# liortalker/MindTheEdge

Measured on AMD Instinct MI355X. Metric: training images/sec, PackNet-SAN+edge-loss 384x1280 bf16, higher is better.
Workload: dtype bf16; 1 GPU; T8: PackNet-SAN + silog + 4-scale depth-edge loss training step, 384x1280, 8 frames/GPU, dropout 0.5, flip 0.5; global_batch=8, height=384, width=1280, parallelism=single GPU

## Files before the change

include/mte_kernels.h:

```cpp
#ifndef MTE_KERNELS_H
#define MTE_KERNELS_H

#ifdef __cplusplus
extern "C" {
#endif

typedef struct ihipStream_t* mte_stream_t;

#define MTE_OK 0
#define MTE_ERR_ARG (-1)
#define MTE_ERR_LAUNCH (-2)
#define MTE_ERR_UNSUPPORTED (-3)
#define MTE_DT_BF16 0
#define MTE_DT_F32 1

#define MTE_CONV_ACCUMULATE 1
#define MTE_CONV_SOLO 2
int mte_conv2d_igemm(const void* x, long ldx, const void* wpack, const float* bias, void* y, long ldy, int out_f32,
                     int B, int H, int W, int Cin_p, int N, int KH, int KW, int dtype,
                     float* workspace, long workspace_elems, int accumulate, mte_stream_t stream);
int mte_conv2d_igemm_unshuffle(const void* x, long ldx, const void* wpack, void* y, long ldy,
                               int B, int H, int W, int Cin_p, int N, int KH, int KW, int dtype, int accumulate, mte_stream_t stream);
#define MTE_OPT_GN_PREZEROED 0
#define MTE_OPT_LOSS_PREZEROED 1
#define MTE_OPT_HANDOFF_FENCES 2
#define MTE_OPT_WGRAD_SHARES_CHIP 3
int mte_set_option(int option, int value);
#define MTE_DEVERR_GN_CLUSTER_FWD 1
#define MTE_DEVERR_GN_CLUSTER_BWD 2
#define MTE_DEVERR_IMAGE_RESAMPLE 4
int mte_device_error_init(void);
int mte_device_error_poll(void);
int mte_conv2d_wgrad(const void* x, long ldx, const void* dy, long ldy, float* dw_stage, int stage_parts, int* parts_out,
                     int B, int H, int W, int Cin_p, int N, int KH, int KW, int dtype, mte_stream_t stream);
int mte_conv2d_wgrad_nine_tap(int H, int W, int Cin_p, int N, int KH, int KW, int dtype);
int mte_pack_conv_weights(const float* w_oihw, void* wfwd, void* wbwd, int Cout, int Cin, int KH, int KW,
                          int Cin_p, int Cout_p, int dtype, mte_stream_t stream);
typedef struct { const float* w; void* wf; void* wb; void* pf; void* pb; int Cout, Cin, taps, Cin_p; int end_f, end_b, end_pf, end_pb; } mte_pack_job;
int mte_pack_conv_weights_multi(const void* jobs, int njobs, int dtype, mte_stream_t stream);
int mte_pack_conv_weights_bwd(const void* wfwd, void* wbwd, int Cout, int KH, int KW, int Cin_p, int dtype, mte_stream_t stream);
int mte_unpack_conv_wgrad(float* dw_stage, int parts, float* dw_oihw, int Cout, int Cin, int KH, int KW, int Cin_p, mte_stream_t stream);
int mte_colsum(const void* y, long ld, long M, int N, float* out, int dtype, mte_stream_t stream);

int mte_conv2d_patch_supported(int W, int Cin_p, int N, int KH, int KW, int dtype);
int mte_conv2d_patch_wgrad_supported(int W, int Cin_p, int N, int KH, int KW, int dtype);
long mte_conv2d_patch_pack_elems(int Cin_p, int N, int KH, int KW);
int mte_conv2d_patch_repack(const void* wgeneric, void* wpatch, int Cin_p, int N, int KH, int KW, mte_stream_t stream);
int mte_conv2d_patch_fwd(const void* x, long ldx, const void* wpatch, const float* bias, void* y, long ldy,
                         int B, int H, int W, int Cin_p, int N, int KH, int KW, int accumulate, mte_stream_t stream);
int mte_conv2d_patch_wgrad(const void* x, long ldx, const void* dy, long lddy, float* dw_stage, int stage_parts, int* parts_out,
                           int B, int H, int W, int Cin_p, int N, int KH, int KW, mte_stream_t stream);
long mte_conv2d_patch_fwd_gn_elems(int B, int H, int W);
int mte_conv2d_patch_fwd_gn(const void* x, long ldx, const void* wpatch, const float* bias, void* y, long ldy, int B, int H, int W, int Cin_p, int N, int KH, int KW,
                            int accumulate, float* rec, long rec_elems, int* tiles_per_sample_out, mte_stream_t stream);

int mte_conv2d_stem_supported(int W, int Cin_p, int N, int KH, int KW, int dtype);
int mte_conv2d_stem_fwd(const void* x, long ldx, const void* wf, const float* bias, void* y, long ldy,
                        int B, int H, int W, int N, int KH, int KW, mte_stream_t stream);
int mte_conv2d_stem_wgrad(const void* x, long ldx, const void* dy, long lddy, float* dw_stage, int stage_parts, int* parts_out,
                          int B, int H, int W, int N, int KH, int KW, mte_stream_t stream);

long mte_gn_stats_elems(int B);
int mte_gn_stats(const void* y1, long ld1, const void* y2, long ld2, const float* scale2, double* stats,
                 int B, int HW, int C, int dtype, mte_stream_t stream);
int mte_gn_stats_from_records(const float* rec, int tiles_per_sample, double* stats, int B, mte_stream_t stream);
int mte_gn_fwd_is_single_pass(int HW, int C, int has_y2, int dtype);
int mte_gn_fwd_is_single_pass_b(int B, int HW, int C, int has_y2, int dtype);
int mte_gn_elu_fwd(const void* y1, long ld1, const void* y2, long ld2, const float* scale2, double* stats, int stats_ready,
                   const float* gamma, const float* beta, void* z, long ldz,
                   int B, int HW, int C, float eps, int dtype, mte_stream_t stream);
int mte_gn_elu_bwd(const void* dz, long lddz, const void* y1, long ld1, const void* y2, long ld2, const float* scale2,
                   const double* stats, const float* gamma, const float* beta, float* red,
                   void* d1, long ldd1, void* d2, long ldd2, float* dgamma, float* dbeta, float* dbias,
                   int B, int HW, int C, float eps, int dtype, mte_stream_t stream);
int mte_gn_tail_fwd(const void* y1, long ld1, const double* stats1, const float* gamma1, const float* beta1,
                    const void* y2, long ld2, const float* scale2, void* t, long ldt, double* stats_t,
                    const float* gamma_t, const float* beta_t, void* z, long ldz,
                    int B, int HW, int C, float eps, int dtype, mte_stream_t stream);

int mte_pack3d_fwd(const void* x, long ldx, const float* w3, const float* b3, void* out, long ldo,
                   int B, int H, int W, int C, int dtype, mte_stream_t stream);
int mte_pack3d_bwd_data(const void* dout, long ldo, const float* w3, void* dx, long lddx,
                        int B, int H, int W, int C, int dtype, mte_stream_t stream);
int mte_pack3d_bwd_weight(const void* x, long ldx, const void* dout, long ldo, float* dwb,
                          int B, int H, int W, int C, int dtype, mte_stream_t stream);
int mte_unpack3d_fwd(const void* x, long ldx, const float* w3, const float* b3, void* out, long ldo,
                     int B, int H, int W, int C, int dtype, mte_stream_t stream);
int mte_unpack3d_bwd_data(const void* dout, long ldo, const float* w3, void* dx, long lddx,
                          int B, int H, int W, int C, int dtype, mte_stream_t stream);
int mte_unpack3d_bwd_weight(const void* x, long ldx, const void* dout, long ldo, float* dwb,
                            int B, int H, int W, int C, int dtype, mte_stream_t stream);

int mte_fold_pack_weights(const float* W, const float* K3, const float* b, const float* b3, float* Wf, float* bf,
                          int Co, int D, int k, mte_stream_t stream);
int mte_unfold_pack_wgrad(const float* dWf, const float* dbf, const float* W, const float* K3, const float* b3,
                          float* dW, float* dk3b, int Co, int D, int k, int accumulate, mte_stream_t stream);
int mte_pixel_shuffle(const void* src, long lds_, void* dst, long ldd, int B, int H, int W, int C, int dir, int dtype, mte_stream_t stream);
int mte_copy_rect(const void* src, long lds_, int Hs, int Ws, int sy, int sx, void* dst, long ldd, int Hd, int Wd, int dy, int dx,
                  int B, int h, int w, int C, int mode, int dtype, mte_stream_t stream);
typedef struct { const void* src; long lds_; int Hs, Ws, sy, sx; void* dst; long ldd; int Hd, Wd, dy, dx, h, w, mode; } mte_rect_op;
int mte_copy_rects(const void* ops, int n, int B, int C, int dtype, mte_stream_t stream);

int mte_invdepth_fwd(const void* x, long ldx, const float* w, const float* bias, float* out,
                     int B, int H, int W, int C, float min_depth, int dtype, mte_stream_t stream);
int mte_invdepth_bwd_data(const float* w, const float* inv_out, const float* dout, float* dlogit,
                          void* dx, long lddx, int B, int H, int W, int C, float min_depth, int dtype, mte_stream_t stream);
long mte_invdepth_bwd_weight_workspace_elems(int C);
int mte_invdepth_bwd_weight(const void* x, long ldx, const float* dlogit, float* dwb, float* records,
                            int B, int H, int W, int C, int dtype, mte_stream_t stream);

int mte_rank1_conv_fwd(const float* inv, const float* w, long w_stride, void* y, long ldy, int B, int h, int wl, int N, int dtype, mte_stream_t stream);
int mte_rank1_conv_bwd_data(const void* dy, long lddy, const float* w, long w_stride, float* dinv, int B, int h, int wl, int N, int accumulate, int dtype,
                            mte_stream_t stream);
int mte_upsample2_f32(const float* inv, float* out, int B, int h, int wl, mte_stream_t stream);
int mte_conv2d_patch_fwd_rank1_ok(const float* bias, long ldx, int B, int H, int W, int Cin_p, int N);
int mte_conv2d_patch_fwd_rank1(const void* x, long ldx, const void* wpatch, const float* bias, void* y, long ldy, int B, int H, int W, int Cin_p, int N,
                               const float* inv, const float* w1, long w1_stride, mte_stream_t stream);
int mte_conv2d_patch_fwd_plus1x1(const void* x, long ldx, const void* wpatch, const float* bias, void* y, long ldy, int B, int H, int W, int Cin_p, int N,
                                 const void* x2, long ldx2, const void* wpatch2, int C2, mte_stream_t stream);
long mte_rank1_conv_bwd_records_elems(int N);
int mte_rank1_conv_bwd_weight(const void* dy, long lddy, const float* inv, float* dw, long dw_stride, float* records,
                              int B, int h, int wl, int N, int dtype, mte_stream_t stream);
int mte_nchw_to_nhwc(const float* src, void* dst, long ldd, int B, int C, int H, int W, int Cp, int flip_w, int dtype, mte_stream_t stream);
int mte_upsample_inv_fwd(const float* inv, void* dst, long ldd, int B, int h, int w, int dtype, mte_stream_t stream);
int mte_upsample_inv_bwd(const void* dsrc, long lds_, float* dinv, int B, int h, int w, int accumulate, int dtype, mte_stream_t stream);
int mte_copy_channels(const void* src, long lds_, void* dst, long ldd, long npix, int C, int dtype, mte_stream_t stream);
int mte_split_record(const float* src, float* dst0, int n0, float* dst1, int n1, mte_stream_t stream);
int mte_add_channels(const void* a, long lda, const void* b, long ldb, void* out, long ldo, long npix, int C, int dtype, mte_stream_t stream);

typedef struct { const float* pred; const float* edge; const float* normal; const float* mask; float* gmap; float* dpred; int H; int W; } mte_edge_scale;
long mte_edge_loss_work_elems(const void* scales, int nscales, int B);
int mte_edge_loss_multi_fwd(const void* scales, int nscales, int B, int from_inv, int is_grad, int is_sigmoid, float thresh,
                            float weight, float pos_to_neg, const float* gt_depth, double* work, float* losses, float* coef,
                            float* silog_loss, float* silog_aux, mte_stream_t stream);
int mte_edge_loss_multi_bwd(const void* scales, int nscales, int B, int from_inv, int is_grad, int is_sigmoid, float thresh,
                            const float* coef, const float* gout, const float* gt_depth, const float* silog_aux, const float* silog_gout,
                            mte_stream_t stream);
typedef struct { const float* pred[2]; float* dpred[2]; const float* edge; const float* normal; int H; int W; } mte_edge_pair_scale;
long mte_edge_loss_pair_work_elems(const void* scales, int nscales, int B);
int mte_edge_loss_pair_fwd(const void* scales, int nscales, int B, float thresh, float weight, float pos_to_neg,
                           const float* gt_depth, double* work, float* losses, float* coef,
                           float* silog_loss, float* silog_aux, mte_stream_t stream);
int mte_edge_loss_pair_bwd(const void* scales, int nscales, int B, float thresh, const float* coef, const float* gout,
                           const float* gt_depth, const float* silog_aux, const float* silog_gout, mte_stream_t stream);
long mte_edge_loss_sums_elems(int B, int H, int W);
int mte_edge_loss_fwd(const float* pred, const float* edge, const float* normal, const float* mask, double* sums, float* gmap,
                      int B, int H, int W, int from_inv, int is_grad, int is_sigmoid, float thresh, mte_stream_t stream);
int mte_edge_loss_finalize(const double* sums, int B, long numel, float weight, float pos_to_neg, int has_mask,
                           float out_scale, float* loss_acc, float* loss_this, float* coef, mte_stream_t stream);
int mte_edge_loss_bwd(const float* pred, const float* edge, const float* normal, const float* mask, const float* coef, const float* gout,
                      float* dpred, int B, int H, int W, int from_inv, int is_grad, int is_sigmoid, float thresh, mte_stream_t stream);

long mte_edge_loss_kind_work_elems(int B, int H, int W);
int mte_edge_loss_kind_fwd(const float* pred, const float* edge, const float* normal, const float* mask, float* gmap, int B, int H, int W,
                           int kind, int dice, int from_inv, int is_grad, int is_sigmoid, float thresh, float weight, float pos_to_neg,
                           double* work, float* loss, float* coef, mte_stream_t stream);
int mte_edge_loss_kind_bwd(const float* pred, const float* edge, const float* normal, const float* mask, const float* coef, const float* gout,
                           float* dpred, int B, int H, int W, int kind, int dice, int from_inv, int is_grad, int is_sigmoid, float thresh,
                           mte_stream_t stream);

typedef struct { const float* pred; float* dpred; int H; int W; } mte_sup_scale;
long mte_supervised_loss_work_elems(const void* scales, int nscales, int B);
int mte_supervised_loss_fwd(const void* scales, int nscales, int B, const float* depth, int Hd, int Wd, int method, int sparse,
                            double* work, float* loss, float* scale_loss, float* coef, mte_stream_t stream);
int mte_supervised_loss_bwd(const void* scales, int nscales, int B, const float* depth, int Hd, int Wd, int method, int sparse,
                            const float* coef, const float* gout, mte_stream_t stream);
typedef struct { const float* src; float* dst; int h; int w; } mte_upsample_map;
int mte_upsample_nearest_fwd(const void* maps, int nmaps, int B, int H, int W, mte_stream_t stream);
int mte_upsample_nearest_bwd(const void* maps, int nmaps, int B, int H, int W, mte_stream_t stream);

int mte_resize_bilinear_fwd(const float* x, float* y, int B, int h, int w, int H, int W, mte_stream_t stream);
int mte_resize_bilinear_bwd(const float* dy, float* dx, int B, int h, int w, int H, int W, mte_stream_t stream);

int mte_silog_fwd(const float* inv, const float* depth, long n, double* sums, float out_scale, float* loss_acc, float* loss_this, float* aux, mte_stream_t stream);
int mte_silog_bwd(const float* inv, const float* depth, const float* aux, const float* gout, float* dinv, long n, int accumulate, mte_stream_t stream);

int mte_adam_step(float* p, const float* g, float* m, float* v, long n, float lr, float beta1, float beta2, float eps,
                  int step, float gscale, mte_stream_t stream);
int mte_adam_step_dev(float* p, const float* g, float* m, float* v, long n, const float* hyper, float beta1, float beta2, float eps,
                      float gscale, mte_stream_t stream);
int mte_adamw_step(float* p, const float* g, float* m, float* v, long n, float lr, float beta1, float beta2, float eps, float weight_decay,
                   int decoupled, int step, float gscale, mte_stream_t stream);
int mte_adamw_step_dev(float* p, const float* g, float* m, float* v, long n, const float* hyper, float beta1, float beta2, float eps,
                       float weight_decay, int decoupled, float gscale, mte_stream_t stream);
int mte_sgd_step(float* p, const float* g, float* buf, long n, float lr, float momentum, float dampening, float weight_decay, int nesterov,
                 int step, float gscale, mte_stream_t stream);
int mte_sgd_step_dev(float* p, const float* g, float* buf, long n, const float* hyper, float momentum, float weight_decay, int nesterov,
                     float gscale, mte_stream_t stream);

long mte_depth_metrics_workspace_bytes(int B);
int mte_depth_metrics(const float* gt, const float* pred, int B, int H, int W, int h, int w, int scale_mode, int garg_crop,
                      float min_depth, float max_depth, int use_gt_scale, void* workspace, long workspace_bytes,
                      float* out7, mte_stream_t stream);
int mte_post_process_inv_depth(const float* inv_depth, const float* inv_depth_flipped, float* out, int B, int H, int W,
                               int method, mte_stream_t stream);

int mte_dee_sobel_nms(const float* pred, float scale, unsigned char* normals_u8, float* nms, int B, int H, int W, mte_stream_t stream);
int mte_hysteresis_begin(const float* img, unsigned char* state, int* info, int B, int H, int W, double t_low, double t_high,
                         mte_stream_t stream);
int mte_hysteresis_propagate(unsigned char* state, int* flags, int sweeps, int B, int H, int W, mte_stream_t stream);
int mte_hysteresis_finish(const float* img, const unsigned char* state, const int* info, float* out, int B, int H, int W,
                          mte_stream_t stream);

long mte_chamfer_workspace_bytes(int B, int H, int W);
int mte_chamfer_distance(const float* im_pred, const float* im_gt, int B, int H, int W, double edge_to_edge_thresh,
                         void* workspace, long workspace_bytes, double* out, float* dist_map, float* cond_map, mte_stream_t stream);

int mte_canny_begin(const float* depth, int B, int H, int W, int n_pairs, const int* thresholds, unsigned* max_ws,
                    unsigned char* vis_u8, unsigned char* state, mte_stream_t stream);
int mte_resize_linear(const float* src, int B, int h, int w, float* dst, int H, int W, mte_stream_t stream);
int mte_canny_propagate(unsigned char* state, int* flags, int sweeps, int maps, int H, int W, mte_stream_t stream);
int mte_canny_finish(const unsigned char* state, float* edges, int maps, int H, int W, mte_stream_t stream);
int mte_canny_begin_fixed(const float* depth, int B, int H, int W, float min_depth, float max_depth, float factor, int n_pairs,
                          const int* thresholds, unsigned char* vis_u8, unsigned char* state, mte_stream_t stream);

long mte_edge_match_workspace_bytes(int B, int H, int W, int r2);
int mte_edge_match(const float* pred, const float* gt, const int* gt_of, int B, int Bg, int H, int W, int r2, const int* init_mate,
                   void* workspace, long workspace_bytes, int* result, int* mate_pred, mte_stream_t stream);

int mte_frame_depth_metrics(const double* gt, const float* pred, const unsigned char* mask_u8, int B, int H, int W,
                            double min_depth, double max_depth, int x0, int x1, int y0, int y1, double* out, long* counts, mte_stream_t stream);

int mte_sparsify_depth(const float* depth, void* feat, long ldf, unsigned char* mask, int B, int H, int W, int dtype, mte_stream_t stream);
long mte_sparse_site_list_workspace_elems(long npix);
int mte_sparse_site_list(const unsigned char* mask, long npix, int* sites, int* count, int* ws, mte_stream_t stream);
int mte_conv2d_igemm_sparse(const void* x, long ldx, const void* wpack, const float* bias, void* y, long ldy,
                            int B, int H, int W, int Cin_p, int N, int KH, int KW, int dtype,
                            const int* sites, const int* count, int accumulate, mte_stream_t stream);
int mte_sparse_maxpool3s2(const void* in, long ldi, const unsigned char* mask_in, void* out, long ldo, unsigned char* mask_out,
                          int B, int H, int W, int C, int dtype, mte_stream_t stream);
int mte_sparse_bn_relu(const void* a, long lda, const void* b, long ldb, const void* c, long ldc, const unsigned char* mask,
                       const float* gamma, const float* beta, const float* mean, const float* var, float eps,
                       void* out, long ldo, long npix, int C, int dtype, mte_stream_t stream);
int mte_san_fuse(const void* skip, long ld_skip, const void* sparse, long ld_sparse, const float* w, const float* bias,
                 void* out, long ldo, long npix, int C, int dtype, mte_stream_t stream);
int mte_sparse_bn_stats(const void* a, long lda, const void* b, long ldb, const void* c, long ldc, const unsigned char* mask,
                        double* sums, long npix, int C, int dtype, mte_stream_t stream);
int mte_sparse_bn_relu_bwd(const void* a, long lda, const void* b, long ldb, const void* c, long ldc, const void* out, long ldo,
                           const void* dout, long ldd, const unsigned char* mask, const float* gamma, const float* mean, const float* invstd,
                           const double* n_active, double* sums, void* dx, long ldx, long npix, int C, int dtype, mte_stream_t stream);
int mte_sparse_maxpool3s2_bwd(const void* in, long ldi, const unsigned char* mask_in, const void* dout, long ldd, void* din, long ldn,
                              int B, int H, int W, int C, int dtype, mte_stream_t stream);
int mte_san_fuse_bwd(const void* skip, long ld_skip, const void* dout, long ldd, const float* w, void* dskip, long ldk, double* sums,
                     long npix, int C, int dtype, mte_stream_t stream);
int mte_feat_l2(const void* a, long lda, const void* b, long ldb, double* sum, void* db, long ldg, const float* gscale, float inv_n,
                long npix, int C, int dtype, mte_stream_t stream);

int mte_edge_target_from_u8(const unsigned char* src, float* dst, long n, mte_stream_t stream);
int mte_normal_target_from_u8(const unsigned char* src, float* dst, long n, mte_stream_t stream);
int mte_resize_depth_preserve(const float* src, int B, int h, int w, float* dst, int H, int W, int* winner_ws, mte_stream_t stream);

int mte_resize_linear_u8(const unsigned char* src, int B, int h, int w, unsigned char* dst, int H, int W, mte_stream_t stream);
int mte_resize_nearest_f32(const float* src, int B, int h, int w, float* dst, int H, int W, mte_stream_t stream);

long mte_image_resample_work_bytes(int in_h, int in_w, int out_h, int out_w, int two_pass);
int mte_image_resample_u8(const unsigned char* src, long src_stride, int crop_x, int crop_y, int in_h, int in_w, unsigned char* dst,
                          int out_h, int out_w, const int* kk_h, const int* bounds_h, int ksize_h, const int* kk_v, const int* bounds_v,
                          int ksize_v, unsigned char* workspace, int two_pass, mte_stream_t stream);
int mte_color_jitter_u8_to_f32(const unsigned char* in, int B, int H, int W, const float* factors, const int* order, int any_contrast,
                               unsigned long long* luma_sums, float* out, float* out_original, mte_stream_t stream);

#define MTE_PREP_EDGE_U8 0
#define MTE_PREP_SPARSE_U16 1
#define MTE_PREP_SPARSE_F32 2
#define MTE_PREP_NORMAL_U8 3
#define MTE_BATCH_PREP_ROW_WORDS 12
int mte_batch_prep(const unsigned char* arena, long arena_bytes, const long* table_host, const long* table_dev, int n_maps, float* out,
                   long out_elems, int* work, long winner_elems, mte_stream_t stream);

long mte_lidar_perturb_work_bytes(int H, int W);
int mte_lidar_index(const float* depth, int H, int W, void* work, mte_stream_t stream);
int mte_lidar_perturb(const float* depth, int H, int W, int n, double scale_d0, const double* add_i, const double* add_j, const double* add_d,
                      void* work, mte_stream_t stream);
int mte_lidar_scatter(int H, int W, int n, const unsigned char* keep, int n_keep, float* out, const void* work, mte_stream_t stream);
int mte_lidar_project(const double* points, int N, const double* K, const float* depth_map, float* out, int H, int W, int* winner_ws,
                      mte_stream_t stream);

long mte_order_stats_work_bytes(int B);
int mte_order_stats_f32(const float* x, long stride, int B, long n, const int* k, int positive_only, float* out, int* count_out, void* work,
                        mte_stream_t stream);
int mte_colormap_u8(const float* x, int B, int H, int W, const float* divisor, const float* lo_hi, const unsigned char* table, unsigned char* out,
                    mte_stream_t stream);
int mte_d3r_count(const float* gt, const float* pred, int H, int W, const void* index_work, int n, const int* pairs, int P, int* count,
                  mte_stream_t stream);

#ifdef MTE_DEV
int mte_debug_set(int key, int value);
#endif

#ifdef __cplusplus
}
#endif
#endif
```

mindtheedge_amd/_build.py:

```python
import hashlib
import os
import subprocess
import sys
from concurrent.futures import ThreadPoolExecutor

CSRC = os.path.join(os.path.dirname(os.path.abspath(__file__)), "csrc")
LIB = os.path.join(CSRC, "libmte_hip.so")
SOURCES = ["conv_igemm.hip", "conv_igemm8.hip", "conv_wgrad9.hip", "tap_wgrad.hip", "conv_patch.hip", "conv_stem.hip", "norm_act.hip", "pack3d.hip", "pack_fold.hip", "heads_misc.hip", "optim.hip", "edge_loss.hip", "edge_loss_kinds.hip", "supervised_loss.hip", "eval_metrics.hip", "dee_post.hip", "chamfer.hip", "canny.hip", "edge_match.hip", "san.hip", "data_prep.hip", "batch_prep.hip", "eval_prep.hip", "image_prep.hip", "lidar_prep.hip", "depth_viz.hip"]
FLAGS = ["--offload-arch=gfx950", "-O3", "-fPIC", "-std=c++17", "-Wno-unused-value", "-ffp-contract=off"]


def _hipcc():
    for c in (os.environ.get("HIPCC"), "/opt/rocm/bin/hipcc", "hipcc"):
        if c and (os.path.isabs(c) and os.path.exists(c) or not os.path.isabs(c)):
            return c
    raise RuntimeError("hipcc not found")


def _digest(paths, extra=""):
    h = hashlib.sha256(extra.encode())
    for p in paths:
        with open(p, "rb") as f:
            h.update(f.read())
    return h.hexdigest()


def _stale(target, digest):
    stamp = target + ".sha256"
    if not (os.path.exists(target) and os.path.exists(stamp)):
        return True
    with open(stamp) as f:
        return f.read().strip() != digest


def _stamp(target, digest):
    with open(target + ".sha256", "w") as f:
        f.write(digest + "\n")


DEV_LIB = os.path.join(CSRC, "libmte_hip_dev.so")


def headers(csrc=CSRC):
    return sorted(os.path.join(csrc, f) for f in os.listdir(csrc) if f.endswith(".hpp"))


def build(force=False, verbose=False, dev=True):
    hipcc = _hipcc()
    hdrs = headers()
    os.makedirs(os.path.join(CSRC, "dev"), exist_ok=True)
    variants = [("", [], LIB)] + ([("dev", ["-DMTE_DEV"], DEV_LIB)] if dev else [])
    jobs = []
    for sub, extra, _ in variants:
        for s in SOURCES:
            src, obj = os.path.join(CSRC, s), os.path.join(CSRC, sub, s.replace(".hip", ".o"))
            dig = _digest([src] + hdrs, " ".join(FLAGS + extra))
            if force or _stale(obj, dig):
                jobs.append(([hipcc] + FLAGS + extra + ["-c", src, "-o", obj], obj, dig))

    def run(cmd):
        if verbose:
            print(" ".join(cmd), file=sys.stderr)
        r = subprocess.run(cmd, capture_output=True, text=True)
        if r.returncode != 0:
            raise RuntimeError("hipcc failed:\n%s\n%s" % (" ".join(cmd), r.stderr[-4000:]))

    def compile_one(job):
        cmd, obj, dig = job
        run(cmd)
        _stamp(obj, dig)

    if jobs:
        with ThreadPoolExecutor(max_workers=min(int(os.environ.get("MTE_BUILD_JOBS", "6")), len(jobs))) as ex:
            list(ex.map(compile_one, jobs))
    for sub, _, target in variants:
        objs = [os.path.join(CSRC, sub, s.replace(".hip", ".o")) for s in SOURCES]
        lib_dig = _digest(objs, "link")
        if force or _stale(target, lib_dig):
            run([hipcc, "--offload-arch=gfx950", "-shared", "-fPIC", "-o", target] + objs)
            _stamp(target, lib_dig)
    return LIB


if __name__ == "__main__":
    print(build(force="--force" in sys.argv, verbose=True))
```

mindtheedge_amd/_lib.py:

```python
import ctypes
import os
import re

_HERE = os.path.dirname(os.path.abspath(__file__))
HEADER = os.path.join(os.path.dirname(_HERE), "include", "mte_kernels.h")
DEV_LIB_PATH = os.path.join(_HERE, "csrc", "libmte_hip_dev.so")
_USE_DEV = bool(os.environ.get("MTE_USE_DEV_LIB"))
LIB_PATH = os.environ.get("MTE_LIB_PATH") or (DEV_LIB_PATH if _USE_DEV else os.path.join(_HERE, "csrc", "libmte_hip.so"))

_CTYPES = {"int": ctypes.c_int, "long": ctypes.c_long, "float": ctypes.c_float, "double": ctypes.c_double, "mte_stream_t": ctypes.c_void_p}
_ERRORS = {-1: "MTE_ERR_ARG (bad argument / unsupported shape)", -2: "MTE_ERR_LAUNCH (HIP launch failed)",
           -3: "MTE_ERR_UNSUPPORTED"}


class MteError(RuntimeError):
    pass


RETURNS = {}
QUERIES = ("mte_conv2d_patch_supported", "mte_conv2d_stem_supported", "mte_conv2d_patch_wgrad_supported", "mte_conv2d_wgrad_nine_tap", "mte_conv2d_patch_fwd_gn_elems", "mte_conv2d_patch_pack_elems", "mte_depth_metrics_workspace_bytes",
           "mte_chamfer_workspace_bytes", "mte_edge_match_workspace_bytes", "mte_edge_loss_sums_elems", "mte_gn_fwd_is_single_pass", "mte_gn_fwd_is_single_pass_b",
           "mte_edge_loss_work_elems", "mte_edge_loss_pair_work_elems", "mte_edge_loss_kind_work_elems", "mte_supervised_loss_work_elems", "mte_rank1_conv_bwd_records_elems", "mte_conv2d_patch_fwd_rank1_ok", "mte_gn_stats_elems", "mte_device_error_poll", "mte_invdepth_bwd_weight_workspace_elems", "mte_sparse_site_list_workspace_elems", "mte_image_resample_work_bytes", "mte_lidar_perturb_work_bytes", "mte_order_stats_work_bytes")


def parse_header(path=HEADER, dev=False):
    text = open(path).read()
    text = re.sub(r"/\*.*?\*/", "", text, flags=re.S)
    if not dev:
        text = re.sub(r"#ifdef MTE_DEV.*?#endif", "", text, flags=re.S)
    protos = {}
    for m in re.finditer(r"\b(int|long)\s+(mte_\w+)\s*\(([^)]*)\)\s*;", text):
        RETURNS[m.group(2)] = ctypes.c_long if m.group(1) == "long" else ctypes.c_int
        args = []
        for a in ([] if m.group(3).strip() in ("", "void") else m.group(3).split(",")):
            a = " ".join(a.split())
            if "*" in a:
                args.append((ctypes.c_void_p, a.split("*")[-1].strip()))
            else:
                ty, name = a.rsplit(" ", 1)
                args.append((_CTYPES[ty.replace("const ", "").strip()], name))
        protos[m.group(2)] = args
    return protos


class _Lib:
    def __init__(self, path=None, dev=None):
        self._dll = None
        self._path = path or LIB_PATH
        self._dev = (self._path == DEV_LIB_PATH) if dev is None else bool(dev)
        self._protos = parse_header(dev=self._dev)
        self._options = {}
        self._loaded = {}

    def load(self):
        if self._dll is None:
            if not os.path.exists(self._path):
                raise MteError("%s is not built (%s). Run `python -c 'import __graft_entry__ as g; g.build()'` "
                               "or `python mindtheedge_amd/_build.py`; there is no CPU/eager fallback." % (os.path.basename(self._path), self._path))
            import torch
            dll = self._loaded.get(self._path)
            if dll is None:
                dll = self._loaded[self._path] = ctypes.CDLL(self._path)
            for name, args in self._protos.items():
                fn = getattr(dll, name)
                fn.argtypes = [t for t, _ in args]
                fn.restype = RETURNS.get(name, ctypes.c_int)
            self._dll = dll
            for opt, val in self._options.items():
                dll.mte_set_option(opt, val)
        return self._dll

    def switch(self, path, dev):
        for k in [k for k in self.__dict__ if k.startswith("mte_")]:
            del self.__dict__[k]
        self._dll, self._path, self._dev = None, path, bool(dev)
        self._protos = parse_header(dev=self._dev)

    def set_option(self, option, value, lazy=False):
        self._options[int(option)] = int(value)
        if not lazy or self._dll is not None:
            self.mte_set_option(int(option), int(value))

    def __getattr__(self, name):
        if name.startswith("mte_"):
            fn = getattr(self.load(), name)
            if name in QUERIES:
                call = fn
            else:
                def call(*args):
                    rc = fn(*args)
                    if rc != 0:
                        raise MteError("%s failed: %s" % (name, _ERRORS.get(rc, rc)))
            self.__dict__[name] = call
            return call
        raise AttributeError(name)


lib = _Lib()


class dev_library:

    def __enter__(self):
        self._prev = (lib._path, lib._dev)
        lib.switch(DEV_LIB_PATH, True)
        return lib

    def __exit__(self, *exc):
        lib.switch(*self._prev)
        return False
```

mindtheedge_amd/kernels.py:

```python
import ctypes
import itertools
import math
import os
import weakref

import torch

from ._lib import lib, MteError

DT_BF16, DT_F32 = 0, 1
_state = {"compute_dtype": torch.bfloat16, "weights_epoch": 0}


def set_compute_dtype(dtype):
    dtype = {"bf16": torch.bfloat16, "fp32": torch.float32, "f32": torch.float32}.get(dtype, dtype)
    assert dtype in (torch.bfloat16, torch.float32)
    _state["compute_dtype"] = dtype


def compute_dtype():
    return _state["compute_dtype"]


def bump_weights_epoch():
    _state["weights_epoch"] += 1


def weights_epoch():
    return _state["weights_epoch"]


class GradSink:

    def __init__(self):
        self.views = {}
        self.on_ready = None
        self.written = set()
        self.announced = set()
        self.suspended = False
        self._suspend_resets = 0

    def register(self, p, view):
        self.views[p.data_ptr()] = view

    def lookup(self, p):
        if self.suspended:
            return None
        key = p.data_ptr()
        v = self.views.get(key)
        if v is not None and key in self.written:
            if key in self.announced and self.on_ready is not None:
                raise MteError("a parameter received a second gradient after its first one was announced to the gradient all-reduce: "
                               "call kernels.suspend_grad_sink() in the forward pass of a graph that uses parameters twice")
            join_side_stream()
            return None
        if v is not None and p.grad is not None and p.grad.data_ptr() == v.data_ptr() and v.shape == p.shape:
            return v
        return None

    def claim(self, p):
        v = self.lookup(p)
        if v is not None:
            self.written.add(p.data_ptr())
        return v

    def reset(self):
        self.written.clear()
        self.announced.clear()
        if self.suspended:
            self._suspend_resets += 1
            if self._suspend_resets >= 2:
                self.suspended = False

    def end_step(self):
        self.suspended = False

    def suspend(self):
        self.suspended = True
        self._suspend_resets = 0

    def ready(self, p):
        self.announced.add(p.data_ptr())
        if self.on_ready is not None:
            self.on_ready(p)


_sink = {"active": None}


def set_grad_sink(sink):
    _sink["active"] = sink


def suspend_grad_sink():
    if _sink["active"] is not None:
        _sink["active"].suspend()


def _grad_dst(p, zero=False):
    sk = _sink["active"]
    if sk is not None:
        v = sk.claim(p)
        if v is not None:
            return v, True
    if zero:
        return _zeros(p.shape, torch.float32, p.device), False
    return torch.empty(p.shape, dtype=torch.float32, device=p.device), False


def _grad_ret(p, t, sunk):
    if sunk:
        _sink["active"].ready(p)
        return None
    return t


def _dt(t):
    if t.dtype == torch.bfloat16:
        return DT_BF16
    if t.dtype == torch.float32:
        return DT_F32
    raise MteError("unsupported activation dtype %s" % t.dtype)


_raw_stream = getattr(torch._C, "_cuda_getCurrentRawStream", None)
_cur_device = getattr(torch._C, "_cuda_getDevice", None)


def _stream():
    if _raw_stream is not None and _cur_device is not None:
        return _raw_stream(_cur_device())
    return torch.cuda.current_stream().cuda_stream


def _require_gpu(t):
    if not t.is_cuda:
        raise MteError("mindtheedge_amd kernels run on an MI355X only; got a %s tensor (no CPU fallback)" % t.device)


def round8(c):
    return (c + 7) // 8 * 8


def new_act(B, C, H, W, dtype=None, device="cuda"):
    return torch.empty_strided((B, C, H, W), (H * W * C, 1, W * C, C), dtype=dtype or compute_dtype(), device=device)


def alias_of(t):
    return torch.empty(0, dtype=t.dtype, device=t.device).set_(t.untyped_storage(), t.storage_offset(), t.size(), t.stride())


def channel_slice(buf, c0, c1):
    return alias_of(buf[:, c0:c1])


def is_act(t):
    if t.dim() != 4 or t.dtype not in (torch.bfloat16, torch.float32):
        return False
    B, C, H, W = t.shape
    sb, sc, sh, sw = t.stride()
    if C > 1 and sc != 1:
        return False
    ld = sw if W > 1 else (sh if H > 1 else (sb if B > 1 else C))
    ok = ld >= C and (H == 1 or W == 1 or sh == W * ld) and (B == 1 or sb == H * W * ld)
    per16 = 8 if t.dtype == torch.bfloat16 else 4
    return bool(ok and ld % per16 == 0 and t.data_ptr() % 16 == 0)


def as_act(t, dtype=None):
    dtype = dtype or t.dtype
    if t.dtype == dtype and is_act(t):
        return t
    out = new_act(t.shape[0], t.shape[1], t.shape[2], t.shape[3], dtype, t.device)
    out.copy_(t)
    return out


def _pl(t):
    if t.dim() == 4:
        B, C, H, W = t.shape
        sb, sc, sh, sw = t.stride()
        if sc == 1 and W > 1 and H > 1 and sh == W * sw and (B == 1 or sb == H * sh) and sw >= C:
            dt = t.dtype
            if (dt is torch.bfloat16 and not (sw & 7)) or (dt is torch.float32 and not (sw & 3)):
                p = t.data_ptr()
                if not (p & 15):
                    return p, sw
    if not is_act(t):
        raise MteError("expected an NHWC activation, got shape %s strides %s" % (tuple(t.shape), t.stride()))
    B, C, H, W = t.shape
    ld = t.stride(3) if W > 1 else (t.stride(2) if H > 1 else (t.stride(0) if B > 1 else C))
    return t.data_ptr(), ld


def _ptr(t):
    return 0 if t is None else t.data_ptr()


_ELEM_SIZE = {torch.float64: 8, torch.float32: 4, torch.bfloat16: 2, torch.float16: 2, torch.uint8: 1, torch.int32: 4, torch.int64: 8}


class _ZeroArena:
    CHUNK = 8 << 20

    def __init__(self):
        self.chunks = {}
        self.captured = []
        self.enabled = False

    def zeros(self, shape, dtype, device):
        if not self.enabled:
            lib.set_option(0, 1)
            lib.set_option(1, 1)
            if os.environ.get("MTE_HANDOFF_FENCES"):
                lib.set_option(2, 1 if os.environ["MTE_HANDOFF_FENCES"] == "1" else 0)
            self.enabled = True
            _device_errors_init()
        n = 1
        for d in shape:
            n *= d
        nbytes = (n * _ELEM_SIZE[dtype] + 255) & ~255
        if nbytes > self.CHUNK // 4:
            return torch.zeros(shape, dtype=dtype, device=device)
        capturing = torch.cuda.is_current_stream_capturing()
        key = (device if isinstance(device, str) else (device.type, device.index), _stream())
        c = self.chunks.get(key)
        if c is None or c[1] + nbytes > self.CHUNK or (capturing and c[2] != self.capture_id) or (not capturing and c[2] is not None):
            if c is not None and c[2] is not None:
                self.captured.append(c[0])
            c = self.chunks[key] = [torch.zeros((self.CHUNK,), dtype=torch.uint8, device=device), 0,
                                    self.capture_id if capturing else None, {}]
        typed = c[3].get(dtype)
        if typed is None:
            typed = c[3][dtype] = c[0].view(dtype)
        strides, acc = [], 1
        for d in reversed(shape):
            strides.append(acc)
            acc *= d
        out = typed.as_strided(shape, strides[::-1], c[1] // _ELEM_SIZE[dtype])
        c[1] += nbytes
        return out

    capture_id = 0

    def begin_capture(self):
        self.capture_id += 1


_arena = _ZeroArena()
_DEVERR_NAMES = {1: "GroupNorm cluster kernel (forward): a workgroup of a cluster never arrived",
                 2: "GroupNorm cluster kernel (backward): a workgroup of a cluster never arrived",
                 4: "image resample: coefficient tables wider than the LANCZOS tables of the given sizes, output tiles left unwritten"}


def _device_errors_init():
    if torch.cuda.is_available() and not torch.cuda.is_current_stream_capturing():
        lib.mte_device_error_init()
        return True
    return False


def check_device_errors():
    code = int(lib.mte_device_error_poll()) if _device_errors_init() else 0
    if code:
        what = "; ".join(v for k, v in _DEVERR_NAMES.items() if code & k) or "code %d" % code
        raise MteError("device error word set (0x%x): %s -- the results of that step are invalid; when this is raised by the optimizer, the parameter "
                       "update of the failed step has already been applied: restore the last checkpoint" % (code, what))


def begin_graph_capture():
    _arena.begin_capture()
    _dropout_pool.clear()


def end_graph_capture():
    _dropout_pool.clear()


def _zeros(shape, dtype, device):
    return _arena.zeros(tuple(shape), dtype, device)


class WeightPack:

    _live = []
    _seq = itertools.count()

    def __init__(self):
        self.key = None
        self.wf = self.wb = None
        self.pf = self.pb = None
        self.pkey = None
        self._last = None
        self._order = -1
        self._event = None
        WeightPack._live.append(weakref.ref(self))

    def _sync_prefetch(self):
        if self._event is not None:
            cur = torch.cuda.current_stream()
            waited = _side.setdefault("last_waited", {})
            if waited.get(cur.cuda_stream) is not self._event:
                cur.wait_event(self._event)
                waited[cur.cuda_stream] = self._event
            self._event = None

    def _patch_pack(self, w, which):
        wf, wb = self.wf, self.wb
        cout, cin, kh, kw = w.shape
        cin_p = round8(cin)
        if which == 'f':
            n = lib.mte_conv2d_patch_pack_elems(cin_p, cout, kh, kw)
            if self.pf is None or self.pf.numel() != n:
                self.pf = torch.empty((n,), dtype=torch.bfloat16, device=w.device)
            lib.mte_conv2d_patch_repack(wf.data_ptr(), self.pf.data_ptr(), cin_p, cout, kh, kw, _stream())
        else:
            n = lib.mte_conv2d_patch_pack_elems(cout, cin_p, kh, kw)
            if self.pb is None or self.pb.numel() != n:
                self.pb = torch.empty((n,), dtype=torch.bfloat16, device=w.device)
            lib.mte_conv2d_patch_repack(wb.data_ptr(), self.pb.data_ptr(), cout, cin_p, kh, kw, _stream())

    def get_patch(self, w, which):
        self.get(w, torch.bfloat16, which == 'b')
        if self.pkey != self.key:
            self.pf_ok = self.pb_ok = False
            self.pkey = self.key
        if which == 'f':
            if not self.pf_ok:
                self._patch_pack(w, 'f')
                self.pf_ok = True
            return self.pf
        if not self.pb_ok:
            self._patch_pack(w, 'b')
            self.pb_ok = True
        return self.pb

    pf_ok = pb_ok = False
    _want_pf = _want_pb = False

    def _pack(self, w, dtype, need_bwd):
        cout, cin, kh, kw = w.shape
        cin_p = round8(cin)
        dtc = DT_BF16 if dtype == torch.bfloat16 else DT_F32
        if self.wf is None or self.wf.dtype != dtype or tuple(self.wf.shape) != (cout, kh * kw, cin_p):
            self.wf = torch.empty((cout, kh * kw, cin_p), dtype=dtype, device=w.device)
            self.wb = None
        if need_bwd and (self.wb is None or self.wb.dtype != dtype):
            self.wb = torch.empty((cin_p, kh * kw, cout), dtype=dtype, device=w.device)
        lib.mte_pack_conv_weights(w.detach().contiguous().data_ptr(), self.wf.data_ptr(), _ptr(self.wb) if need_bwd else 0,
                                  cout, cin, kh, kw, cin_p, cout, dtc, _stream())
        self.has_bwd = bool(need_bwd)

    has_bwd = False

    def get(self, w, dtype, need_bwd):
        key = (w.data_ptr(), w._version, weights_epoch(), dtype, tuple(w.shape))
        self._last = (weakref.ref(w), dtype)
        self._order = next(WeightPack._seq)
        if key != self.key:
            if self._event is not None:
                torch.cuda.current_stream().wait_event(self._event)
            self._event = None
            self._pack(w, dtype, need_bwd)
            self.key = key
        else:
            self._sync_prefetch()
            if need_bwd and not self.has_bwd:
                cout, cin, kh, kw = w.shape
                cin_p = round8(cin)
                if self.wb is None:
                    self.wb = torch.empty((cin_p, kh * kw, cout), dtype=dtype, device=w.device)
                lib.mte_pack_conv_weights_bwd(self.wf.data_ptr(), self.wb.data_ptr(), cout, kh, kw, cin_p,
                                              DT_BF16 if dtype == torch.bfloat16 else DT_F32, _stream())
                self.has_bwd = True
        return self.wf, (self.wb if self.has_bwd else None)


class _PackJob(ctypes.Structure):
    _fields_ = [("w", ctypes.c_void_p), ("wf", ctypes.c_void_p), ("wb", ctypes.c_void_p), ("pf", ctypes.c_void_p), ("pb", ctypes.c_void_p),
                ("Cout", ctypes.c_int), ("Cin", ctypes.c_int), ("taps", ctypes.c_int), ("Cin_p", ctypes.c_int),
                ("end_f", ctypes.c_int), ("end_b", ctypes.c_int), ("end_pf", ctypes.c_int), ("end_pb", ctypes.c_int)]


_PACK_CHUNKS = (16, 48)
_pack_jobs = {"sig": None, "chunks": []}


def _pack_job_chunks(packs):
    sig = (len(packs),) + tuple((id(pk), pk._last[0]().data_ptr(), pk.wf.data_ptr(), _ptr(pk.wb) if pk.has_bwd else 0,
                                 _ptr(pk.pf) if pk._want_pf else 0, _ptr(pk.pb) if pk._want_pb else 0) for pk in packs)
    if _pack_jobs["sig"] == sig:
        return _pack_jobs["chunks"]
    chunks = []
    for dt in (torch.bfloat16, torch.float32):
        part = [pk for pk in packs if pk._last[1] == dt and pk.wf is not None and pk.wf.dtype == dt]
        i = 0
        while i < len(part):
            group = part[i:i + (_PACK_CHUNKS[0] if i == 0 else _PACK_CHUNKS[1])]
            i += len(group)
            arr = (_PackJob * len(group))()
            for o, pk in zip(arr, group):
                w = pk._last[0]()
                cout, cin, kh, kw = w.shape
                o.w, o.wf = w.data_ptr(), pk.wf.data_ptr()
                o.wb = pk.wb.data_ptr() if pk.has_bwd else None
                o.pf = pk.pf.data_ptr() if pk._want_pf else None
                o.pb = pk.pb.data_ptr() if pk._want_pb else None
                o.Cout, o.Cin, o.taps, o.Cin_p = cout, cin, kh * kw, round8(cin)
            chunks.append((arr, len(group), DT_BF16 if dt == torch.bfloat16 else DT_F32, group))
    _pack_jobs["sig"], _pack_jobs["chunks"] = sig, chunks
    return chunks


def prefetch_weight_packs():
    packs = []
    for r in WeightPack._live:
        pk = r()
        if pk is not None and pk._last is not None and pk.key is not None and pk._last[0]() is not None and pk._last[0]().is_cuda:
            packs.append(pk)
    WeightPack._live = [r for r in WeightPack._live if r() is not None]
    if not packs:
        return
    packs.sort(key=lambda pk: pk._order)
    if _side["enabled"]:
        if not _side["streams"]:
            _side["streams"] = [_new_side_stream() for _ in range(max(1, _SIDE_STREAMS))]
        side = _side["streams"][0]
        ev = torch.cuda.Event()
        ev.record()
        side.wait_event(ev)
    else:
        side = torch.cuda.current_stream()
    with torch.cuda.stream(side):
        _refold_all()
        _refresh_main_weights(packs)
        for pk in packs:
            pk._want_pf = pk.pf_ok and pk.pkey == pk.key and pk.pf is not None
            pk._want_pb = pk.pb_ok and pk.pkey == pk.key and pk.pb is not None and pk.has_bwd
        st = _stream()
        odd = [pk for pk in packs if not (pk._last[0]().is_contiguous() and pk._last[0]().dtype == torch.float32)]
        if odd:
            packs = [pk for pk in packs if pk not in odd]
            for pk in odd:
                w, dtype = pk._last[0](), pk._last[1]
                pk._pack(w, dtype, pk.has_bwd)
                pk.key = (w.data_ptr(), w._version, weights_epoch(), dtype, tuple(w.shape))
                pk.pkey, pk.pf_ok, pk.pb_ok, pk._event = None, False, False, None
        for arr, n, dtc, group in _pack_job_chunks(packs):
            lib.mte_pack_conv_weights_multi(ctypes.addressof(arr), n, dtc, st)
            ev = None
            if _side["enabled"]:
                ev = torch.cuda.Event()
                ev.record(side)
            for pk in group:
                w, dtype = pk._last[0](), pk._last[1]
                pk.key = (w.data_ptr(), w._version, weights_epoch(), dtype, tuple(w.shape))
                pk.pkey = pk.key
                pk.pf_ok, pk.pb_ok = pk._want_pf, pk._want_pb
                pk._event = ev
    if _side["enabled"] and torch.cuda.is_current_stream_capturing():
        torch.cuda.current_stream().wait_stream(side)
        for pk in packs:
            pk._event = None


SPLITK_SLABS = 8
_splitk_ws = {}


def _splitk_workspace(M, N, device):
    tiles = ((M + 127) // 128) * ((N + 127) // 128)
    if tiles >= 384:
        return None, 0
    n = SPLITK_SLABS * M * N
    if torch.cuda.is_current_stream_capturing():
        return torch.empty((n,), dtype=torch.float32, device=device), n
    key = (str(device), _stream())
    ws = _splitk_ws.get(key)
    if ws is None or ws.numel() < n:
        ws = _splitk_ws[key] = torch.empty((n,), dtype=torch.float32, device=device)
    return ws, n


_cfg = {"patch_kernels": True, "pack_folding": True, "pack_fold_max_overhead": 0.30,
        "no_fork_accumulate": bool(os.environ.get("MTE_NO_FORK_ACCUM")),
        "patch_wgrad_slabs": not os.environ.get("MTE_PATCH_WGRAD_ATOMICS"),
        "split_inv_channel": os.environ.get("MTE_SPLIT_INV", "1") == "1",
        "fuse_inv_term": os.environ.get("MTE_FUSE_INV", "1") == "1",
        "fold_shortcut_dgrad": os.environ.get("MTE_FOLD_SHORTCUT", "1") == "1",
        "fuse_residual_tail": os.environ.get("MTE_FUSE_TAIL", "1") == "1",
        "gn_stats_in_conv": os.environ.get("MTE_GN_IN_CONV", "1") == "1"}



def use_pack_folding(flag):
    _cfg["pack_folding"] = bool(flag)


def pack_folding_enabled():
    return _cfg["pack_folding"]


def use_patch_kernels(flag):
    _cfg["patch_kernels"] = bool(flag)


def _stem_ok(W, cin_p, n, kh, kw, dtype):
    return (_cfg["patch_kernels"] and cin_p == 8 and dtype == torch.bfloat16
            and lib.mte_conv2d_stem_supported(W, cin_p, n, kh, kw, DT_BF16) == 1)


def _patch_ok(W, cin_p, n, kh, kw, dtype):
    return _cfg["patch_kernels"] and dtype == torch.bfloat16 and lib.mte_conv2d_patch_supported(W, cin_p, n, kh, kw, DT_BF16) == 1


class SiteList:

    def __init__(self, mask):
        _require_gpu(mask)
        if mask.dtype != torch.uint8 or not mask.is_contiguous():
            raise MteError("site list: expected a contiguous uint8 mask [B,H,W]")
        n = mask.numel()
        self.rows = torch.empty((n,), dtype=torch.int32, device=mask.device)
        self.count = torch.empty((1,), dtype=torch.int32, device=mask.device)
        ws = torch.empty((int(lib.mte_sparse_site_list_workspace_elems(n)),), dtype=torch.int32, device=mask.device)
        lib.mte_sparse_site_list(mask.data_ptr(), n, self.rows.data_ptr(), self.count.data_ptr(), ws.data_ptr(), _stream())
        self.shape = tuple(mask.shape)


def conv_forward(x, wf, bias, cout, kh, kw, out=None, pack=None, w=None, accumulate=False, sites=None, gn_records=None):
    B, Cp, H, W = x.shape
    if out is None:
        out = new_act(B, cout, H, W, x.dtype, x.device)
        if sites is not None:
            out.zero_()
    xp, ldx = _pl(x)
    yp, ldy = _pl(out)
    if sites is not None:
        if sites.shape != (B, H, W):
            raise MteError("site list of a %s mask used on a %s map" % (sites.shape, (B, H, W)))
        lib.mte_conv2d_igemm_sparse(xp, ldx, wf.data_ptr(), _ptr(bias), yp, ldy, B, H, W, Cp, cout, kh, kw, _dt(x),
                                    sites.rows.data_ptr(), sites.count.data_ptr(), 1 if accumulate else 0, _stream())
        return out
    if not accumulate and _stem_ok(W, Cp, cout, kh, kw, x.dtype):
        lib.mte_conv2d_stem_fwd(xp, ldx, wf.data_ptr(), _ptr(bias), yp, ldy, B, H, W, cout, kh, kw, _stream())
        return out
    if pack is not None and _patch_ok(W, Cp, cout, kh, kw, x.dtype):
        if (gn_records is not None and _cfg["gn_stats_in_conv"] and cout % 16 == 0
                and lib.mte_gn_fwd_is_single_pass_b(B, H * W, cout, 0, _dt(x)) != 1):
            n = int(lib.mte_conv2d_patch_fwd_gn_elems(B, H, W))
            rec = torch.empty((n,), dtype=torch.float32, device=x.device)
            tiles = ctypes.c_int(0)
            lib.mte_conv2d_patch_fwd_gn(xp, ldx, pack.get_patch(w, 'f').data_ptr(), _ptr(bias), yp, ldy, B, H, W, Cp, cout, kh, kw,
                                        1 if accumulate else 0, rec.data_ptr(), n, ctypes.byref(tiles), _stream())
            gn_records.append((rec, tiles.value))
            return out
        lib.mte_conv2d_patch_fwd(xp, ldx, pack.get_patch(w, 'f').data_ptr(), _ptr(bias), yp, ldy, B, H, W, Cp, cout, kh, kw,
                                 1 if accumulate else 0, _stream())
        return out
    ws, ws_n = _splitk_workspace(B * H * W, cout, x.device)
    lib.mte_conv2d_igemm(xp, ldx, wf.data_ptr(), _ptr(bias), yp, ldy, 0, B, H, W, Cp, cout, kh, kw, _dt(x), _ptr(ws), ws_n,
                         (1 if accumulate else 0) | _CONV_SOLO, _stream())
    return out


_CONV_SOLO = 2


_side = {"enabled": True, "streams": [], "next": 0, "keep": [], "keep_bytes": 0, "callback_queued": False, "dirty": False}
lib.set_option(3, 1, lazy=True)
def _new_side_stream():
    pr = int(os.environ.get("MTE_SIDE_PRIORITY", "1"))
    if pr == 0:
        return torch.cuda.Stream()
    hip = ctypes.CDLL("libamdhip64.so")
    h = ctypes.c_void_p()
    if hip.hipStreamCreateWithPriority(ctypes.byref(h), 1, pr) != 0:
        raise RuntimeError("hipStreamCreateWithPriority(%d) failed" % pr)
    return torch.cuda.ExternalStream(h.value)


_SIDE_STREAMS = 1
_SIDE_KEEP_LIMIT = 24 << 30


def use_wgrad_side_stream(flag):
    _side["enabled"] = bool(flag)
    lib.set_option(3, 1 if flag else 0, lazy=True)


class _BandChain:

    def __enter__(self):
        return self

    def __exit__(self, *exc):
        return False

    def mark(self):
        return None

    def join(self, ev=None):
        return None


def join_side_stream():
    if _side["dirty"]:
        for st in _side["streams"]:
            ev = torch.cuda.Event()
            ev.record(st)
            torch.cuda.current_stream().wait_event(ev)
        _side["dirty"] = False
    _side["keep"].clear()
    _side["keep_bytes"] = 0


def side_streams_wait_into(stream):
    if _side["dirty"]:
        for st in _side["streams"]:
            ev = torch.cuda.Event()
            ev.record(st)
            stream.wait_event(ev)


def _side_join_callback():
    _side["callback_queued"] = False
    join_side_stream()


def _side_stream_for(*tensors):
    if not _side["streams"]:
        _side["streams"] = [_new_side_stream() for _ in range(max(1, _SIDE_STREAMS))]
    side = _side["streams"][_side["next"] % len(_side["streams"])]
    _side["next"] += 1
    ev = torch.cuda.Event()
    ev.record()
    side.wait_event(ev)
    _side["keep"].append(tensors)
    _side["keep_bytes"] += sum(t.numel() * t.element_size() for t in tensors)
    _side["dirty"] = True
    if not _side["callback_queued"]:
        try:
            torch.autograd.Variable._execution_engine.queue_callback(_side_join_callback)
            _side["callback_queued"] = True
        except RuntimeError:
            pass
    return side


def _conv_wgrad(x, dy, w, need_dbias, dw_out, dbias_out):
    cout, cin, kh, kw = w.shape
    B, Cp, H, W = x.shape
    dyp, lddy = _pl(dy)
    xp, ldx = _pl(x)
    st = _stream()
    dbias = None
    per = cout * kh * kw * Cp
    patch = _cfg["patch_kernels"] and x.dtype == torch.bfloat16 and lib.mte_conv2d_patch_wgrad_supported(W, Cp, cout, kh, kw, DT_BF16) == 1
    if patch and lib.mte_conv2d_wgrad_nine_tap(H, W, Cp, cout, kh, kw, _dt(x)) == 1:
        patch = False
    if kh * kw == 1 and Cp >= 64:
        patch = False
    wide = 256 if per <= (1 << 18) else (64 if per <= (1 << 19) else 32)
    cap = max(1, min(512, (192 << 20) // (4 * per))) if patch and _cfg["patch_wgrad_slabs"] else max(1, min(wide, (96 << 20) // (4 * per)))
    stem = _stem_ok(W, Cp, cout, kh, kw, x.dtype)
    if stem:
        cap = 2048
    stage = torch.empty((cap + (32 if cap > 32 else 0), cout, kh * kw, Cp), dtype=torch.float32, device=x.device)
    parts = ctypes.c_int(1)
    if stem:
        lib.mte_conv2d_stem_wgrad(xp, ldx, dyp, lddy, stage.data_ptr(), cap, ctypes.byref(parts), B, H, W, cout, kh, kw, st)
    elif patch:
        lib.mte_conv2d_patch_wgrad(xp, ldx, dyp, lddy, stage.data_ptr(), cap, ctypes.byref(parts), B, H, W, Cp, cout, kh, kw, st)
    else:
        lib.mte_conv2d_wgrad(xp, ldx, dyp, lddy, stage.data_ptr(), cap, ctypes.byref(parts), B, H, W, Cp, cout, kh, kw, _dt(x), st)
    dw = dw_out if dw_out is not None else torch.empty_like(w, dtype=torch.float32)
    lib.mte_unpack_conv_wgrad(stage.data_ptr(), parts.value, dw.data_ptr(), cout, cin, kh, kw, Cp, st)
    if need_dbias:
        dbias = dbias_out if dbias_out is not None else torch.empty((cout,), dtype=torch.float32, device=x.device)
        lib.mte_colsum(dyp, lddy, B * H * W, cout, dbias.data_ptr(), _dt(dy), st)
    return dw, dbias


def conv_backward(x, dy, w, pack, need_dx, need_dw=True, need_dbias=True, dw_out=None, dbias_out=None, fork_slot=None, sunk=False, sites=None):
    dw = dbias = dx = None
    on_side = False
    if need_dw:
        sunk = bool(sunk) and dw_out is not None and (dbias_out is not None or not need_dbias)
        on_side = sunk and _side["enabled"] and need_dx

    def wgrad():
        if on_side:
            if _side["keep_bytes"] > _SIDE_KEEP_LIMIT:
                join_side_stream()
            with torch.cuda.stream(_side_stream_for(x, dy)):
                return _conv_wgrad(x, dy, w, need_dbias, dw_out, dbias_out)
        return _conv_wgrad(x, dy, w, need_dbias, dw_out, dbias_out)

    if need_dw:
        dw, dbias = wgrad()
    if need_dx:
        dx = _conv_dgrad(x, dy, w, pack, fork_slot, sites)
    return dx, dw, dbias


def _conv_dgrad(x, dy, w, pack, fork_slot, sites):
    cout, cin, kh, kw = w.shape
    B, Cp, H, W = x.shape
    dyp, lddy = _pl(dy)
    st = _stream()
    target = _fork_target(fork_slot, (B, Cp, H, W), x.dtype, keep_pending=True)
    if (target is None and fork_slot is not None and (kh, kw) == (1, 1) and sites is None and _cfg["fold_shortcut_dgrad"]
            and not _cfg.get("no_fork_accumulate") and _patch_ok(W, cout, Cp, 1, 1, x.dtype) and _patch_ok(W, 32, Cp, 3, 3, x.dtype)):
        dx = new_act(B, Cp, H, W, x.dtype, x.device)
        fork_slot["buf"] = dx
        fork_slot["pending"] = (dy, w, pack)
        return dx
    pend = _pending_slot(fork_slot) if target is not None else None
    if pend is not None:
        dy3, w3, pack3 = pend["pending"]
        if ((kh, kw) == (3, 3) and sites is None and target is pend["buf"] and _patch_ok(W, cout, Cp, 3, 3, x.dtype)
                and tuple(dy3.shape[2:]) == (H, W) and dy3.dtype == x.dtype):
            del pend["pending"]
            d3p, ldd3 = _pl(dy3)
            dxp, lddx = _pl(target)
            lib.mte_conv2d_patch_fwd_plus1x1(dyp, lddy, pack.get_patch(w, 'b').data_ptr(), 0, dxp, lddx, B, H, W, cout, Cp,
                                             d3p, ldd3, pack3.get_patch(w3, 'b').data_ptr(), dy3.shape[1], st)
            fork_slot["buf"] = target
            return target
        _flush_pending(pend)
    dx = target if target is not None else new_act(B, Cp, H, W, x.dtype, x.device)
    if target is None and sites is not None:
        dx.zero_()
    acc = 1 if target is not None else 0
    dxp, lddx = _pl(dx)
    if sites is not None:
        _, wb = pack.get(w, x.dtype, True)
        lib.mte_conv2d_igemm_sparse(dyp, lddy, wb.data_ptr(), 0, dxp, lddx, B, H, W, cout, Cp, kh, kw, _dt(x),
                                    sites.rows.data_ptr(), sites.count.data_ptr(), acc, st)
    elif _patch_ok(W, cout, Cp, kh, kw, x.dtype):
        lib.mte_conv2d_patch_fwd(dyp, lddy, pack.get_patch(w, 'b').data_ptr(), 0, dxp, lddx, B, H, W, cout, Cp, kh, kw, acc, st)
    else:
        _, wb = pack.get(w, x.dtype, True)
        ws, ws_n = _splitk_workspace(B * H * W, Cp, x.device)
        lib.mte_conv2d_igemm(dyp, lddy, wb.data_ptr(), 0, dxp, lddx, 0, B, H, W, cout, Cp, kh, kw, _dt(x), _ptr(ws), ws_n, acc, st)
    if fork_slot is not None:
        fork_slot["buf"] = dx
    return dx


_stats_elems = {}


def gn_stats_buffer(B, device):
    n = _stats_elems.get(B)
    if n is None:
        n = _stats_elems[B] = int(lib.mte_gn_stats_elems(B))
    return _zeros((n,), torch.float64, device)


def _gn_forward(y1, y2, scale2, gamma, beta, eps, out=None, records=None):
    B, C, H, W = y1.shape
    p1, l1 = _pl(y1)
    p2, l2 = _pl(y2) if y2 is not None else (0, 0)
    st = _stream()
    ready = 1
    stats = gn_stats_buffer(B, y1.device)
    if lib.mte_gn_fwd_is_single_pass_b(B, H * W, C, 1 if y2 is not None else 0, _dt(y1)) == 1:
        ready = 0
    elif records and y2 is None:
        lib.mte_gn_stats_from_records(records[0][0].data_ptr(), records[0][1], stats.data_ptr(), B, st)
    else:
        lib.mte_gn_stats(p1, l1, p2, l2, _ptr(scale2), stats.data_ptr(), B, H * W, C, _dt(y1), st)
    z = out if out is not None else new_act(B, C, H, W, y1.dtype, y1.device)
    if tuple(z.shape) != (B, C, H, W) or z.dtype != y1.dtype:
        raise MteError("output destination has shape %s / %s, expected %s / %s" % (tuple(z.shape), z.dtype, (B, C, H, W), y1.dtype))
    zp, lz = _pl(z)
    lib.mte_gn_elu_fwd(p1, l1, p2, l2, _ptr(scale2), stats.data_ptr(), ready, gamma.data_ptr(), beta.data_ptr(), zp, lz,
                       B, H * W, C, eps, _dt(y1), st)
    return z, stats


def _gn_backward(dz, y1, y2, scale2, stats, gamma, beta, eps, need_d2, want_dbias=False, dgamma=None, dbeta=None, dbias=None):
    B, C, H, W = y1.shape
    dz = as_act(dz, y1.dtype)
    red = _zeros((B, C, 2), torch.float32, y1.device)
    d1 = new_act(B, C, H, W, y1.dtype, y1.device)
    d2 = new_act(B, C, H, W, y1.dtype, y1.device) if need_d2 else None
    dgamma = dgamma if dgamma is not None else _zeros((C,), torch.float32, y1.device)
    dbeta = dbeta if dbeta is not None else _zeros((C,), torch.float32, y1.device)
    if want_dbias and dbias is None:
        dbias = _zeros((C,), torch.float32, y1.device)
    pz, lz = _pl(dz)
    p1, l1 = _pl(y1)
    p2, l2 = _pl(y2) if y2 is not None else (0, 0)
    pd1, ld1 = _pl(d1)
    pd2, ld2 = _pl(d2) if d2 is not None else (0, 0)
    lib.mte_gn_elu_bwd(pz, lz, p1, l1, p2, l2, _ptr(scale2), stats.data_ptr(), gamma.data_ptr(), beta.data_ptr(), red.data_ptr(),
                       pd1, ld1, pd2, ld2, dgamma.data_ptr(), dbeta.data_ptr(), _ptr(dbias), B, H * W, C, eps, _dt(y1), _stream())
    if want_dbias:
        return d1, d2, dgamma, dbeta, dbias
    return d1, d2, dgamma, dbeta


GN_EPS = 1e-5

_dropout_pool = {}


def dropout2d_scale(B, C, p, device):
    key = (str(device), float(p))
    pool = _dropout_pool.get(key)
    n = B * C
    if pool is None or pool[1] + n > pool[0].numel():
        size = max(1 << 17, 2 * n)
        pool = _dropout_pool[key] = [(torch.rand((size,), device=device) >= p).float() / (1.0 - p), 0]
    out = pool[0][pool[1]:pool[1] + n].view(B, C)
    pool[1] += n
    return out



class ConvGnEluFn(torch.autograd.Function):

    @staticmethod
    def forward(ctx, x, w, b, gamma, beta, pack, out=None):
        ctx.fork_slot = getattr(x, "_mte_fork_slot", None)
        wf, _ = pack.get(w, x.dtype, bool(ctx.needs_input_grad[0]))
        cout, cin, kh, kw = w.shape
        recs = []
        y = conv_forward(x, wf, b, cout, kh, kw, pack=pack, w=w, gn_records=recs)
        z, stats = _gn_forward(y, None, None, gamma, beta, GN_EPS, out=None if out is None else alias_of(out), records=recs)
        ctx.save_for_backward(x, w, y, stats, gamma, beta)
        ctx.pack = pack
        ctx.bias = b
        return z

    @staticmethod
    def backward(ctx, dz):
        x, w, y, stats, gamma, beta = ctx.saved_tensors
        b = ctx.bias
        gg, sg = _grad_dst(gamma, zero=True)
        gb, sb = _grad_dst(beta, zero=True)
        gbias, sbias = _grad_dst(b, zero=True)
        gw, sw = _grad_dst(w)
        dy, _, dgamma, dbeta, db = _gn_backward(dz, y, None, None, stats, gamma, beta, GN_EPS, False, want_dbias=True,
                                                dgamma=gg, dbeta=gb, dbias=gbias)
        dx, dw, _ = conv_backward(x, dy, w, ctx.pack, ctx.needs_input_grad[0], need_dbias=False, dw_out=gw, fork_slot=ctx.fork_slot, sunk=sw)
        return dx, _grad_ret(w, dw, sw), _grad_ret(b, db, sbias), _grad_ret(gamma, dgamma, sg), _grad_ret(beta, dbeta, sb), None, None


def _main_weight(pack, w, cm):
    key = (w.data_ptr(), w._version, weights_epoch())
    wm = getattr(pack, "_main_w", None)
    if wm is None or tuple(wm.shape) != (w.shape[0], cm, w.shape[2], w.shape[3]) or wm.device != w.device:
        wm = pack._main_w = torch.empty((w.shape[0], cm, w.shape[2], w.shape[3]), dtype=torch.float32, device=w.device)
        pack._main_key = None
    pack._main_src = (weakref.ref(w), cm)
    if pack._main_key != key:
        wm.copy_(w.detach()[:, :cm])
        pack._main_key = key
    return wm


def _refresh_main_weights(packs):
    for pk in packs:
        src = getattr(pk, "_main_src", None)
        wm = getattr(pk, "_main_w", None)
        if src is None or wm is None:
            continue
        w = src[0]()
        if w is None or tuple(wm.shape) != (w.shape[0], src[1], w.shape[2], w.shape[3]):
            continue
        key = (w.data_ptr(), w._version, weights_epoch())
        if pk._main_key != key:
            wm.copy_(w.detach()[:, :src[1]])
            pk._main_key = key


class ConvGnEluInvFn(torch.autograd.Function):

    @staticmethod
    def forward(ctx, x, inv, w, b, gamma, beta, pack, out=None):
        ctx.fork_slot = getattr(x, "_mte_fork_slot", None)
        cout, cin, kh, kw = w.shape
        cm = cin - 1
        B, Cp, H, W = x.shape
        if (kh, kw) != (3, 3) or Cp != cm or tuple(inv.shape) != (B, 1, H // 2, W // 2):
            raise MteError("rank-1 inverse-depth term: expected a 3x3 layer over %d + 1 channels and a [B,1,H/2,W/2] map, got %s / %s / %s"
                           % (Cp, tuple(w.shape), tuple(x.shape), tuple(inv.shape)))
        wm = _main_weight(pack, w, cm)
        wf, _ = pack.get(wm, x.dtype, bool(ctx.needs_input_grad[0]))
        invc = inv.detach().contiguous().float()
        y = new_act(B, cout, H, W, x.dtype, x.device)
        yp, ldy = _pl(y)
        w1 = w.detach().data_ptr() + 4 * cm * 9
        xp, ldx = _pl(x)
        if (_cfg["fuse_inv_term"] and pack is not None and _patch_ok(W, Cp, cout, kh, kw, x.dtype)
                and lib.mte_conv2d_patch_fwd_rank1_ok(_ptr(b), ldx, B, H, W, Cp, cout) == 1):
            lib.mte_conv2d_patch_fwd_rank1(xp, ldx, pack.get_patch(wm, 'f').data_ptr(), _ptr(b), yp, ldy, B, H, W, Cp, cout,
                                           invc.data_ptr(), w1, cin * 9, _stream())
        else:
            lib.mte_rank1_conv_fwd(invc.data_ptr(), w1, cin * 9, yp, ldy, B, H // 2, W // 2, cout, _dt(y), _stream())
            conv_forward(x, wf, b, cout, kh, kw, out=y, pack=pack, w=wm, accumulate=True)
        z, stats = _gn_forward(y, None, None, gamma, beta, GN_EPS, out=None if out is None else alias_of(out))
        ctx.save_for_backward(x, invc, w, wm, y, stats, gamma, beta)
        ctx.pack = pack
        ctx.bias = b
        return z

    @staticmethod
    def backward(ctx, dz):
        x, invc, w, wm, y, stats, gamma, beta = ctx.saved_tensors
        b = ctx.bias
        cout, cin, kh, kw = w.shape
        cm = cin - 1
        B, Cp, H, W = x.shape
        gg, sg = _grad_dst(gamma, zero=True)
        gb, sb = _grad_dst(beta, zero=True)
        gbias, sbias = _grad_dst(b, zero=True)
        gw, sw = _grad_dst(w)
        dy, _, dgamma, dbeta, db = _gn_backward(dz, y, None, None, stats, gamma, beta, GN_EPS, False, want_dbias=True,
                                                dgamma=gg, dbeta=gb, dbias=gbias)
        dyp, lddy = _pl(dy)

        dinv = torch.empty((B, 1, H // 2, W // 2), dtype=torch.float32, device=x.device)
        wl = w.detach()
        lib.mte_rank1_conv_bwd_data(dyp, lddy, wl.data_ptr() + 4 * cm * 9, cin * 9, dinv.data_ptr(), B, H // 2, W // 2, cout, 0, _dt(dy), _stream())

        def weight_gradients():
            dwm, _ = _conv_wgrad(x, dy, wm, False, None, None)
            gw[:, :cm].copy_(dwm)
            rec = torch.empty((int(lib.mte_rank1_conv_bwd_records_elems(cout)),), dtype=torch.float32, device=x.device)
            lib.mte_rank1_conv_bwd_weight(dyp, lddy, invc.data_ptr(), gw.data_ptr() + 4 * cm * 9, cin * 9, rec.data_ptr(), B, H // 2, W // 2, cout, _dt(dy), _stream())

        if sw and _side["enabled"]:
            if _side["keep_bytes"] > _SIDE_KEEP_LIMIT:
                join_side_stream()
            with torch.cuda.stream(_side_stream_for(x, dy, invc)):
                weight_gradients()
        else:
            weight_gradients()
        dx = None
        if ctx.needs_input_grad[0]:
            dx = conv_backward(x, dy, wm, ctx.pack, True, need_dw=False, need_dbias=False, fork_slot=ctx.fork_slot)[0]
        if not ctx.needs_input_grad[1]:
            dinv = None
        return dx, dinv, _grad_ret(w, gw, sw), _grad_ret(b, db, sbias), _grad_ret(gamma, dgamma, sg), _grad_ret(beta, dbeta, sb), None, None


class ConvFn(torch.autograd.Function):

    @staticmethod
    def forward(ctx, x, w, b, pack, bias_grad=True):
        ctx.fork_slot = getattr(x, "_mte_fork_slot", None)
        wf, _ = pack.get(w, x.dtype, bool(ctx.needs_input_grad[0]))
        cout, cin, kh, kw = w.shape
        y = conv_forward(x, wf, b, cout, kh, kw, pack=pack, w=w)
        ctx.save_for_backward(x, w)
        ctx.pack = pack
        ctx.bias = b
        ctx.bias_grad = bool(bias_grad)
        return y

    @staticmethod
    def backward(ctx, dy):
        x, w = ctx.saved_tensors
        b = ctx.bias
        dy = as_act(dy, x.dtype)
        gw, sw = _grad_dst(w)
        if not ctx.bias_grad:
            dx, dw, _ = conv_backward(x, dy, w, ctx.pack, ctx.needs_input_grad[0], need_dbias=False, dw_out=gw, fork_slot=ctx.fork_slot, sunk=sw)
            return dx, _grad_ret(w, dw, sw), None, None, None
        gbias, sbias = _grad_dst(b)
        dx, dw, db = conv_backward(x, dy, w, ctx.pack, ctx.needs_input_grad[0], dw_out=gw, dbias_out=gbias, fork_slot=ctx.fork_slot,
                                   sunk=sw and sbias)
        return dx, _grad_ret(w, dw, sw), _grad_ret(b, db, sbias), None, None


class ResidualTailFn(torch.autograd.Function):

    @staticmethod
    def forward(ctx, a, s, scale, gamma, beta, bias_s=None):
        z, stats = _gn_forward(a, s, scale, gamma, beta, GN_EPS)
        ctx.save_for_backward(a, s, stats, gamma, beta)
        ctx.scale = scale
        ctx.bias_s = bias_s
        return z

    @staticmethod
    def backward(ctx, dz):
        a, s, stats, gamma, beta = ctx.saved_tensors
        gg, sg = _grad_dst(gamma, zero=True)
        gb, sb = _grad_dst(beta, zero=True)
        if ctx.bias_s is not None and ctx.needs_input_grad[5]:
            gbs, sbs = _grad_dst(ctx.bias_s, zero=True)
            da, ds, dgamma, dbeta, dbs = _gn_backward(dz, a, s, ctx.scale, stats, gamma, beta, GN_EPS, True, want_dbias=True,
                                                      dgamma=gg, dbeta=gb, dbias=gbs)
            return da, ds, None, _grad_ret(gamma, dgamma, sg), _grad_ret(beta, dbeta, sb), _grad_ret(ctx.bias_s, dbs, sbs)
        da, ds, dgamma, dbeta = _gn_backward(dz, a, s, ctx.scale, stats, gamma, beta, GN_EPS, True, dgamma=gg, dbeta=gb)
        return da, ds, None, _grad_ret(gamma, dgamma, sg), _grad_ret(beta, dbeta, sb), None


def residual_tail_fused_ok(B, C, H, W, dtype):
    if not _cfg["fuse_residual_tail"]:
        return False
    return lib.mte_gn_fwd_is_single_pass_b(B, H * W, C, 1, DT_BF16 if dtype == torch.bfloat16 else DT_F32) != 1


class ConvResidualTailFn(torch.autograd.Function):

    @staticmethod
    def forward(ctx, x1, w2, b2, gamma2, beta2, pack2, s, scale, gamma_t, beta_t, bias_s):
        ctx.fork_slot = getattr(x1, "_mte_fork_slot", None)
        wf, _ = pack2.get(w2, x1.dtype, bool(ctx.needs_input_grad[0]))
        cout, cin, kh, kw = w2.shape
        recs = []
        c2 = conv_forward(x1, wf, b2, cout, kh, kw, pack=pack2, w=w2, gn_records=recs)
        B, C, H, W = c2.shape
        if tuple(s.shape) != (B, C, H, W) or s.dtype != c2.dtype:
            raise MteError("residual tail: shortcut %s / %s against %s / %s" % (tuple(s.shape), s.dtype, (B, C, H, W), c2.dtype))
        st = _stream()
        p1, l1 = _pl(c2)
        p2, l2 = _pl(s)
        stats2 = gn_stats_buffer(B, c2.device)
        if recs:
            lib.mte_gn_stats_from_records(recs[0][0].data_ptr(), recs[0][1], stats2.data_ptr(), B, st)
        else:
            lib.mte_gn_stats(p1, l1, 0, 0, 0, stats2.data_ptr(), B, H * W, C, _dt(c2), st)
        stats_t = gn_stats_buffer(B, c2.device)
        t = new_act(B, C, H, W, c2.dtype, c2.device)
        z = new_act(B, C, H, W, c2.dtype, c2.device)
        pt, lt = _pl(t)
        pz, lz = _pl(z)
        lib.mte_gn_tail_fwd(p1, l1, stats2.data_ptr(), gamma2.data_ptr(), beta2.data_ptr(), p2, l2, _ptr(scale), pt, lt, stats_t.data_ptr(),
                            gamma_t.data_ptr(), beta_t.data_ptr(), pz, lz, B, H * W, C, GN_EPS, _dt(c2), st)
        ctx.save_for_backward(x1, w2, c2, stats2, gamma2, beta2, t, stats_t, gamma_t, beta_t)
        ctx.scale = scale
        ctx.bias_s = bias_s
        ctx.bias2 = b2
        ctx.pack = pack2
        return z

    @staticmethod
    def backward(ctx, dz):
        x1, w2, c2, stats2, gamma2, beta2, t, stats_t, gamma_t, beta_t = ctx.saved_tensors
        scale, bias_s, b2 = ctx.scale, ctx.bias_s, ctx.bias2
        ggt, sgt = _grad_dst(gamma_t, zero=True)
        gbt, sbt = _grad_dst(beta_t, zero=True)
        want_bs = bias_s is not None and ctx.needs_input_grad[10]
        gbs, sbs = _grad_dst(bias_s, zero=True) if want_bs else (None, False)
        if scale is None:
            out = _gn_backward(dz, t, None, None, stats_t, gamma_t, beta_t, GN_EPS, False, want_dbias=want_bs, dgamma=ggt, dbeta=gbt, dbias=gbs)
            dt = ds = out[0]
        else:
            out = _gn_backward(dz, t, None, scale, stats_t, gamma_t, beta_t, GN_EPS, True, want_dbias=want_bs, dgamma=ggt, dbeta=gbt, dbias=gbs)
            dt, ds = out[0], out[1]
        dgamma_t, dbeta_t = out[2], out[3]
        dbs = out[4] if want_bs else None
        gg2, sg2 = _grad_dst(gamma2, zero=True)
        gb2, sb2 = _grad_dst(beta2, zero=True)
        gbias2, sbias2 = _grad_dst(b2, zero=True)
        gw2, sw2 = _grad_dst(w2)
        dc2, _, dgamma2, dbeta2, db2 = _gn_backward(dt, c2, None, None, stats2, gamma2, beta2, GN_EPS, False, want_dbias=True,
                                                    dgamma=gg2, dbeta=gb2, dbias=gbias2)
        dx1, dw2, _ = conv_backward(x1, dc2, w2, ctx.pack, ctx.needs_input_grad[0], need_dbias=False, dw_out=gw2, fork_slot=ctx.fork_slot, sunk=sw2)
        return (dx1, _grad_ret(w2, dw2, sw2), _grad_ret(b2, db2, sbias2), _grad_ret(gamma2, dgamma2, sg2), _grad_ret(beta2, dbeta2, sb2), None,
                ds if ctx.needs_input_grad[6] else None, None, _grad_ret(gamma_t, dgamma_t, sgt), _grad_ret(beta_t, dbeta_t, sbt),
                _grad_ret(bias_s, dbs, sbs) if want_bs else None)


class Pack3dFn(torch.autograd.Function):

    @staticmethod
    def forward(ctx, x, w3, b3):
        B, C, H, W = x.shape
        out = new_act(B, 16 * C, H // 2, W // 2, x.dtype, x.device)
        xp, ldx = _pl(x)
        op, ldo = _pl(out)
        w3c, b3c = w3.detach().contiguous().float(), b3.detach().contiguous().float()
        lib.mte_pack3d_fwd(xp, ldx, w3c.data_ptr(), b3c.data_ptr(), op, ldo, B, H, W, C, _dt(x), _stream())
        ctx.save_for_backward(x, w3c)
        ctx.params = (w3, b3)
        return out

    @staticmethod
    def backward(ctx, dout):
        x, w3c = ctx.saved_tensors
        B, C, H, W = x.shape
        dout = as_act(dout, x.dtype)
        dop, ldo = _pl(dout)
        dw3, db3 = _conv3d_weight_grads(lib.mte_pack3d_bwd_weight, x, dout, *ctx.params)
        dx = None
        if ctx.needs_input_grad[0]:
            dx = new_act(B, C, H, W, x.dtype, x.device)
            dxp, lddx = _pl(dx)
            lib.mte_pack3d_bwd_data(dop, ldo, w3c.data_ptr(), dxp, lddx, B, H, W, C, _dt(x), _stream())
        return dx, dw3, db3


class Unpack3dFn(torch.autograd.Function):

    @staticmethod
    def forward(ctx, x, w3, b3, out=None):
        B, C, H, W = x.shape
        out = alias_of(out) if out is not None else new_act(B, C, 2 * H, 2 * W, x.dtype, x.device)
        if tuple(out.shape) != (B, C, 2 * H, 2 * W) or out.dtype != x.dtype:
            raise MteError("unpack destination has shape %s, expected %s" % (tuple(out.shape), (B, C, 2 * H, 2 * W)))
        xp, ldx = _pl(x)
        op, ldo = _pl(out)
        w3c, b3c = w3.detach().contiguous().float(), b3.detach().contiguous().float()
        lib.mte_unpack3d_fwd(xp, ldx, w3c.data_ptr(), b3c.data_ptr(), op, ldo, B, H, W, C, _dt(x), _stream())
        ctx.save_for_backward(x, w3c)
        ctx.params = (w3, b3)
        return out

    @staticmethod
    def backward(ctx, dout):
        x, w3c = ctx.saved_tensors
        B, C, H, W = x.shape
        dout = as_act(dout, x.dtype)
        dop, ldo = _pl(dout)
        dw3, db3 = _conv3d_weight_grads(lib.mte_unpack3d_bwd_weight, x, dout, *ctx.params)
        dx = new_act(B, C, H, W, x.dtype, x.device)
        dxp, lddx = _pl(dx)
        lib.mte_unpack3d_bwd_data(dop, ldo, w3c.data_ptr(), dxp, lddx, B, H, W, C, _dt(x), _stream())
        return dx, dw3, db3, None


def _rect(src, sy, sx, dst, dy, dx, h, w, mode=0):
    B, C, Hd, Wd = dst.shape
    dp, ldd = _pl(dst)
    if mode == 2:
        lib.mte_copy_rect(0, 0, 0, 0, 0, 0, dp, ldd, Hd, Wd, dy, dx, B, h, w, C, 2, _dt(dst), _stream())
        return
    sp, lds_ = _pl(src)
    lib.mte_copy_rect(sp, lds_, src.shape[2], src.shape[3], sy, sx, dp, ldd, Hd, Wd, dy, dx, B, h, w, C, mode, _dt(dst), _stream())


class _RectOp(ctypes.Structure):
    _fields_ = [("src", ctypes.c_void_p), ("lds_", ctypes.c_long), ("Hs", ctypes.c_int), ("Ws", ctypes.c_int), ("sy", ctypes.c_int),
                ("sx", ctypes.c_int), ("dst", ctypes.c_void_p), ("ldd", ctypes.c_long), ("Hd", ctypes.c_int), ("Wd", ctypes.c_int),
                ("dy", ctypes.c_int), ("dx", ctypes.c_int), ("h", ctypes.c_int), ("w", ctypes.c_int), ("mode", ctypes.c_int)]


def _rects(ops):
    arr = (_RectOp * len(ops))()
    B = C = dt = None
    for o, (src, sy, sx, dst, dy, dx, h, w, mode) in zip(arr, ops):
        Bd, Cd, Hd, Wd = dst.shape
        if B is None:
            B, C, dt = Bd, Cd, _dt(dst)
        elif (Bd, Cd, _dt(dst)) != (B, C, dt):
            raise MteError("rectangle batch: mixed batch / channel / dtype")
        dp, ldd = _pl(dst)
        o.dst, o.ldd, o.Hd, o.Wd, o.dy, o.dx, o.h, o.w, o.mode = dp, ldd, Hd, Wd, dy, dx, h, w, mode
        if mode != 2:
            sp, lds_ = _pl(src)
            o.src, o.lds_, o.Hs, o.Ws, o.sy, o.sx = sp, lds_, src.shape[2], src.shape[3], sy, sx
    lib.mte_copy_rects(ctypes.addressof(arr), len(ops), B, C, dt, _stream())


def _deliver(p, t):
    sk = _sink["active"]
    if sk is not None:
        v = sk.claim(p)
        if v is not None:
            v.copy_(t.view(v.shape))
            sk.ready(p)
            return None
    return t


def _deliver_pair(w, b, rec, nw):
    sk = _sink["active"]
    if sk is not None:
        vw, vb = sk.lookup(w), sk.lookup(b)
        if vw is not None and vb is not None and vw.is_contiguous() and vb.is_contiguous() and vw.numel() == nw and vb.numel() == rec.numel() - nw:
            sk.claim(w)
            sk.claim(b)
            lib.mte_split_record(rec.data_ptr(), vw.data_ptr(), nw, vb.data_ptr(), rec.numel() - nw, _stream())
            sk.ready(w)
            sk.ready(b)
            return None, None
    return _deliver(w, rec[:nw].view(w.shape)), _deliver(b, rec[nw:])


def _claim_adjacent(*params):
    sk = _sink["active"]
    if sk is None:
        return None
    views = [sk.lookup(p) for p in params]
    if any(v is None or not v.is_contiguous() or v.dtype != torch.float32 for v in views):
        return None
    ptr = views[0].data_ptr()
    for v in views:
        if v.data_ptr() != ptr:
            return None
        ptr += 4 * v.numel()
    for p in params:
        sk.claim(p)
    return views[0].as_strided((sum(v.numel() for v in views),), (1,))


def _announce(*params):
    for p in params:
        _sink["active"].ready(p)


def _all_sunk(*params):
    sk = _sink["active"]
    return sk is not None and all(sk.lookup(p) is not None for p in params)


def _conv3d_weight_grads(kernel, x, dout, w3, b3):
    B, C, H, W = x.shape

    def run():
        dop, ldo = _pl(dout)
        xp, ldx = _pl(x)
        dst = _claim_adjacent(w3, b3)
        dwb = dst if dst is not None else torch.empty((112,), dtype=torch.float32, device=x.device)
        kernel(xp, ldx, dop, ldo, dwb.data_ptr(), B, H, W, C, _dt(x), _stream())
        if dst is not None:
            _announce(w3, b3)
            return None, None
        return _deliver_pair(w3, b3, dwb, 108)

    if _side["enabled"] and _all_sunk(w3, b3):
        with torch.cuda.stream(_side_stream_for(x, dout)):
            return run()
    return run()


def pack_fold_applicable(H2, W2, k):
    hb = 2 * (k // 2) + 1
    return H2 > 2 * hb and W2 > 2 * hb and (2.0 * hb / H2 + 2.0 * hb / W2) <= _cfg["pack_fold_max_overhead"]


def _fold_key(w, w3, b, b3):
    return (weights_epoch(), w.data_ptr(), w._version, w3.data_ptr(), w3._version, b.data_ptr(), b._version, b3.data_ptr(), b3._version)


def _fold_now(f, w, w3, b, b3):
    co, C4, k = f["geom"]
    lib.mte_fold_pack_weights(w.detach().data_ptr(), w3.detach().contiguous().float().data_ptr(), b.detach().data_ptr(),
                              b3.detach().contiguous().float().data_ptr(), f["Wf"].data_ptr(), f["bf"].data_ptr(), co, C4, k, _stream())
    f["key"] = _fold_key(w, w3, b, b3)


def _folded_weights(pack_fold, w, w3, b, b3, co, C, k, dev):
    f = getattr(pack_fold, "fold", None)
    if f is None or f["geom"] != (co, 4 * C, k) or f["Wf"].device != dev:
        f = pack_fold.fold = {"geom": (co, 4 * C, k), "key": None,
                              "Wf": torch.empty((co, 4 * C, k + 2, k + 2), dtype=torch.float32, device=dev),
                              "bf": torch.empty((co,), dtype=torch.float32, device=dev)}
        _fold_hooks.append(weakref.ref(pack_fold))
    f["params"] = tuple(weakref.ref(t) for t in (w, w3, b, b3))
    if f["key"] != _fold_key(w, w3, b, b3) or _FOLD_INLINE:
        _fold_now(f, w, w3, b, b3)
        pack_fold.key = None
    return f["Wf"], f["bf"]


_FOLD_INLINE = bool(os.environ.get("MTE_FOLD_INLINE"))
_fold_hooks = []


def _refold_all():
    live = []
    for r in _fold_hooks:
        pk = r()
        f = getattr(pk, "fold", None) if pk is not None else None
        if f is None:
            continue
        live.append(r)
        ps = [p() for p in f.get("params", ())]
        if len(ps) == 4 and all(p is not None for p in ps) and f["key"] != _fold_key(*ps):
            _fold_now(f, *ps)
    _fold_hooks[:] = live


_unshuffle_ok = {}


def _dgrad_unshuffled(dy, Wf, pack, dx, k):
    B, C, H, W = dx.shape
    cp = dy.shape[1]
    if dy.dtype != torch.bfloat16 or 4 * C > 256 or os.environ.get("MTE_NO_UNSHUFFLE") == "1":
        return False
    key = (B, H // 2, W // 2, cp, 4 * C, k)
    ok = _unshuffle_ok.get(key)
    if ok is False:
        return False
    _, wb = pack.get(Wf, dy.dtype, True)
    dyp, lddy = _pl(dy)
    dxp, lddx = _pl(dx)
    args = (dyp, lddy, wb.data_ptr(), dxp, lddx, B, H // 2, W // 2, cp, 4 * C, k, k, _dt(dy), 0, _stream())
    if ok is None:
        from . import _lib as _L
        rc = _L.lib.load().mte_conv2d_igemm_unshuffle(*args)
        if rc not in (0, -3):
            raise MteError("mte_conv2d_igemm_unshuffle failed: %s" % rc)
        _unshuffle_ok[key] = rc == 0
        return rc == 0
    lib.mte_conv2d_igemm_unshuffle(*args)
    return True


class PackFoldedConvGnEluFn(torch.autograd.Function):

    @staticmethod
    def forward(ctx, x, w3, b3, w, b, gamma, beta, pack_unf, pack_fold, out=None):
        B, C, H, W = x.shape
        H2, W2 = H // 2, W // 2
        co, _, k, _ = w.shape
        pad, hb = k // 2, 2 * (k // 2) + 1
        dt, dev = _dt(x), x.device
        w3c, b3c = w3.detach().contiguous().float(), b3.detach().contiguous().float()
        bands = _BandChain()
        with bands:
            wu, _ = pack_unf.get(w, x.dtype, False)
            xb1 = new_act(2 * B, C, 2 * hb, W, x.dtype, dev)
            xb2 = new_act(2 * B, C, H, 2 * hb, x.dtype, dev)
            _rects([(x, 0, 0, xb1[:B], 0, 0, 2 * hb, W, 0), (x, H - 2 * hb, 0, xb1[B:], 0, 0, 2 * hb, W, 0),
                    (x, 0, 0, xb2[:B], 0, 0, H, 2 * hb, 0), (x, 0, W - 2 * hb, xb2[B:], 0, 0, H, 2 * hb, 0)])
            Tb = []
            for xb, (hh, ww) in ((xb1, (hb, W2)), (xb2, (H2, hb))):
                T = new_act(2 * B, 16 * C, hh, ww, x.dtype, dev)
                sp, lds_ = _pl(xb)
                tp, ldt = _pl(T)
                lib.mte_pack3d_fwd(sp, lds_, w3c.data_ptr(), b3c.data_ptr(), tp, ldt, 2 * B, xb.shape[2], xb.shape[3], C, dt, _stream())
                Tb.append(T)
            yb1 = conv_forward(Tb[0], wu, b, co, k, k, pack=pack_unf, w=w)
            yb2 = conv_forward(Tb[1], wu, b, co, k, k, pack=pack_unf, w=w)
        P = new_act(B, 4 * C, H2, W2, x.dtype, dev)
        xp, ldx = _pl(x)
        pp, ldp = _pl(P)
        lib.mte_pixel_shuffle(xp, ldx, pp, ldp, B, H, W, C, 0, dt, _stream())
        Wf, bf = _folded_weights(pack_fold, w, w3, b, b3, co, C, k, dev)
        wfp, _ = pack_fold.get(Wf, x.dtype, False)
        y = conv_forward(P, wfp, bf, co, k + 2, k + 2, pack=pack_fold, w=Wf)
        bands.join()
        _rects([(yb1[:B], 0, 0, y, 0, 0, pad, W2, 0), (yb1[B:], hb - pad, 0, y, H2 - pad, 0, pad, W2, 0),
                (yb2[:B], pad, 0, y, pad, 0, H2 - 2 * pad, pad, 0), (yb2[B:], pad, hb - pad, y, pad, W2 - pad, H2 - 2 * pad, pad, 0)])
        z, stats = _gn_forward(y, None, None, gamma, beta, GN_EPS, out=None if out is None else alias_of(out))
        ctx.save_for_backward(P, xb1, xb2, Tb[0], Tb[1], y, stats, w, w3c, b3c, gamma, beta, Wf)
        ctx.params = (w3, b3, b)
        ctx.packs = (pack_unf, pack_fold)
        ctx.geom = (B, C, H, W, co, k)
        return z

    @staticmethod
    def backward(ctx, dz):
        P, xb1, xb2, T1, T2, y, stats, w, w3c, b3c, gamma, beta, Wf = ctx.saved_tensors
        w3, b3, b = ctx.params
        pack_unf, pack_fold = ctx.packs
        B, C, H, W, co, k = ctx.geom
        H2, W2, pad, hb = H // 2, W // 2, k // 2, 2 * (k // 2) + 1
        dt, dev = _dt(P), P.device
        gg, sg = _grad_dst(gamma, zero=True)
        gbt, sbt = _grad_dst(beta, zero=True)
        dy, _, dgamma, dbeta = _gn_backward(dz, y, None, None, stats, gamma, beta, GN_EPS, False, dgamma=gg, dbeta=gbt)
        bands = _BandChain()
        with bands:
            dyb1 = torch.zeros((2 * B, hb, W2, co), dtype=P.dtype, device=dev).permute(0, 3, 1, 2)
            dyb2 = torch.zeros((2 * B, H2, hb, co), dtype=P.dtype, device=dev).permute(0, 3, 1, 2)
            _rects([(dy, 0, 0, dyb1[:B], 0, 0, pad, W2, 0), (dy, H2 - pad, 0, dyb1[B:], hb - pad, 0, pad, W2, 0),
                    (dy, pad, 0, dyb2[:B], pad, 0, H2 - 2 * pad, pad, 0), (dy, pad, W2 - pad, dyb2[B:], pad, hb - pad, H2 - 2 * pad, pad, 0)])
            gathered = bands.mark()
            dTs, dxb = [], []
            for xb, T, dyb in ((xb1, T1, dyb1), (xb2, T2, dyb2)):
                dT, _, _ = conv_backward(T, dyb, w, pack_unf, True, need_dw=False)
                Bb, _, hx, wx = xb.shape
                tp, ldt = _pl(dT)
                dxi = new_act(Bb, C, hx, wx, P.dtype, dev)
                dp_, ldd = _pl(dxi)
                lib.mte_pack3d_bwd_data(tp, ldt, w3c.data_ptr(), dp_, ldd, Bb, hx, wx, C, dt, _stream())
                dTs.append(dT)
                dxb.append(dxi)
        bands.join(gathered)
        _rects([(None, 0, 0, dy, 0, 0, pad, W2, 2), (None, 0, 0, dy, H2 - pad, 0, pad, W2, 2),
                (None, 0, 0, dy, pad, 0, H2 - 2 * pad, pad, 2), (None, 0, 0, dy, pad, W2 - pad, H2 - 2 * pad, pad, 2)])

        def weight_grads():
            bands.join()
            sw = _stream()
            dw_band = db_band = None
            dst3 = _claim_adjacent(w3, b3)
            dk3b = dst3 if dst3 is not None else torch.zeros((112,), dtype=torch.float32, device=dev)
            gw_dst, gw_sunk = _grad_dst(w)
            gb_dst, gb_sunk = _grad_dst(b)
            for xb, T, dyb, dT in ((xb1, T1, dyb1, dTs[0]), (xb2, T2, dyb2, dTs[1])):
                dwi, dbi = _conv_wgrad(T, dyb, w, True, gw_dst if dw_band is None else None, None)
                dw_band = dwi if dw_band is None else dw_band.add_(dwi)
                db_band = dbi if db_band is None else db_band.add_(dbi)
                Bb, _, hx, wx = xb.shape
                tmp = torch.empty((112,), dtype=torch.float32, device=dev)
                sp, lds_ = _pl(xb)
                tp, ldt = _pl(dT)
                lib.mte_pack3d_bwd_weight(sp, lds_, tp, ldt, tmp.data_ptr(), Bb, hx, wx, C, dt, sw)
                dk3b.add_(tmp)
            dWf, dbf = _conv_wgrad(P, dy, Wf, True, None, None)
            lib.mte_unfold_pack_wgrad(dWf.data_ptr(), dbf.data_ptr(), w.detach().data_ptr(), w3c.data_ptr(), b3c.data_ptr(),
                                      dw_band.data_ptr(), dk3b.data_ptr(), co, 4 * C, k, 1, sw)
            db = torch.add(dbf, db_band, out=gb_dst)
            if dst3 is not None:
                _announce(w3, b3)
                g3 = gb3 = None
            else:
                g3, gb3 = _deliver_pair(w3, b3, dk3b, 108)
            return (g3, gb3, _grad_ret(w, dw_band, gw_sunk), _grad_ret(b, db, gb_sunk))

        if _side["enabled"] and _all_sunk(w3, b3, w, b):
            with torch.cuda.stream(_side_stream_for(P, dy, T1, T2, dyb1, dyb2, dTs[0], dTs[1], xb1, xb2, Wf)):
                g3, gb3, gw, gb = weight_grads()
        else:
            g3, gb3, gw, gb = weight_grads()
        dx = new_act(B, C, H, W, P.dtype, dev)
        if not _dgrad_unshuffled(dy, Wf, pack_fold, dx, k + 2):
            dP, _, _ = conv_backward(P, dy, Wf, pack_fold, True, need_dw=False)
            sp, lds_ = _pl(dP)
            dp_, ldd = _pl(dx)
            lib.mte_pixel_shuffle(sp, lds_, dp_, ldd, B, H, W, C, 1, dt, _stream())
        bands.join()
        _rects([(dxb[0][:B], 0, 0, dx, 0, 0, 2 * hb, W, 1), (dxb[0][B:], 0, 0, dx, H - 2 * hb, 0, 2 * hb, W, 1)])
        _rects([(dxb[1][:B], 0, 0, dx, 0, 0, H, 2 * hb, 1), (dxb[1][B:], 0, 0, dx, 0, W - 2 * hb, H, 2 * hb, 1)])
        return (dx, g3, gb3, gw, gb, _grad_ret(gamma, dgamma, sg), _grad_ret(beta, dbeta, sbt), None, None, None)


class InvDepthFn(torch.autograd.Function):

    @staticmethod
    def forward(ctx, x, w, b, min_depth):
        B, C, H, W = x.shape
        out = torch.empty((B, 1, H, W), dtype=torch.float32, device=x.device)
        xp, ldx = _pl(x)
        wc = w.detach().contiguous().float()
        lib.mte_invdepth_fwd(xp, ldx, wc.data_ptr(), b.detach().float().data_ptr(), out.data_ptr(), B, H, W, C, min_depth, _dt(x), _stream())
        ctx.save_for_backward(x, wc, out)
        ctx.min_depth = min_depth
        ctx.params = (w, b)
        return out

    @staticmethod
    def backward(ctx, dout):
        x, wc, out = ctx.saved_tensors
        w, b = ctx.params
        B, C, H, W = x.shape
        dout = dout.contiguous().float()
        dx = new_act(B, C, H, W, x.dtype, x.device)
        dlogit = torch.empty((B, H, W), dtype=torch.float32, device=x.device)
        dxp, lddx = _pl(dx)
        lib.mte_invdepth_bwd_data(wc.data_ptr(), out.data_ptr(), dout.data_ptr(), dlogit.data_ptr(), dxp, lddx,
                                  B, H, W, C, ctx.min_depth, _dt(x), _stream())

        def weight_grads():
            xp, ldx = _pl(x)
            dst = _claim_adjacent(w, b) if tuple(w.shape) == (1, C, 3, 3) and b.numel() == 1 else None
            dwb = dst if dst is not None else torch.empty((C * 9 + 1,), dtype=torch.float32, device=x.device)
            rec = torch.empty((int(lib.mte_invdepth_bwd_weight_workspace_elems(C)),), dtype=torch.float32, device=x.device)
            lib.mte_invdepth_bwd_weight(xp, ldx, dlogit.data_ptr(), dwb.data_ptr(), rec.data_ptr(), B, H, W, C, _dt(x), _stream())
            if dst is not None:
                _announce(w, b)
                return None, None
            return _deliver_pair(w, b, dwb, C * 9)

        if _side["enabled"] and _all_sunk(w, b):
            with torch.cuda.stream(_side_stream_for(x, dlogit)):
                dw, db = weight_grads()
        else:
            dw, db = weight_grads()
        return dx, dw, db, None


def _pending_slot(slot):
    while slot is not None:
        if slot["buf"] is not None:
            return slot if "pending" in slot else None
        slot = slot["parent"]
    return None


def _flush_pending(slot):
    dy3, w3, pack3 = slot.pop("pending")
    dx = slot["buf"]
    B, Cp, H, W = dx.shape
    cout = w3.shape[0]
    d3p, ldd3 = _pl(dy3)
    dxp, lddx = _pl(dx)
    lib.mte_conv2d_patch_fwd(d3p, ldd3, pack3.get_patch(w3, 'b').data_ptr(), 0, dxp, lddx, B, H, W, cout, Cp, 1, 1, 0, _stream())


def _fork_target(slot, shape, dtype, keep_pending=False):
    if _cfg.get("no_fork_accumulate"):
        return None
    while slot is not None:
        buf = slot["buf"]
        if buf is not None:
            if "pending" in slot and not keep_pending:
                _flush_pending(slot)
            return buf if (tuple(buf.shape) == tuple(shape) and buf.dtype == dtype and is_act(buf)) else None
        slot = slot["parent"]
    return None


class ForkFn(torch.autograd.Function):

    @staticmethod
    def forward(ctx, x, slot):
        ctx.slot = slot
        return alias_of(x), alias_of(x)

    @staticmethod
    def backward(ctx, g1, g2):
        slot = ctx.slot
        if "pending" in slot:
            _flush_pending(slot)
        if g1 is None or g2 is None:
            out = g1 if g2 is None else g2
        elif g1.data_ptr() == g2.data_ptr() and g1.shape == g2.shape and g1.stride() == g2.stride():
            out = g1
        else:
            dt = g1.dtype if g1.dtype == g2.dtype else compute_dtype()
            g1, g2 = as_act(g1, dt), as_act(g2, dt)
            B, C, H, W = g1.shape
            out = new_act(B, C, H, W, dt, g1.device)
            p1, l1 = _pl(g1)
            p2, l2 = _pl(g2)
            po, lo = _pl(out)
            lib.mte_add_channels(p1, l1, p2, l2, po, lo, B * H * W, C, _dt(out), _stream())
        slot["buf"] = None
        return out, None


def fork(x):
    if not (torch.is_grad_enabled() and x.requires_grad):
        return x, x
    slot = {"buf": None, "parent": getattr(x, "_mte_fork_slot", None)}
    a, b = ForkFn.apply(x, slot)
    a._mte_fork_slot = slot
    b._mte_fork_slot = slot
    return a, b


class ConcatFn(torch.autograd.Function):

    @staticmethod
    def forward(ctx, inv, buf, *parts):
        B, _, H, W = parts[0].shape
        dtype = parts[0].dtype
        chans = [p.shape[1] for p in parts]
        ctot = sum(chans) + (8 if inv is not None else 0)
        if buf is None:
            buf = new_act(B, ctot, H, W, dtype, parts[0].device)
        else:
            if tuple(buf.shape) != (B, ctot, H, W) or buf.dtype != dtype:
                raise MteError("concat buffer has shape %s, expected %s" % (tuple(buf.shape), (B, ctot, H, W)))
            buf = alias_of(buf)
        st = _stream()
        off = 0
        for p, c in zip(parts, chans):
            dst = buf[:, off:off + c]
            off += c
            if p.dtype == dtype and p.data_ptr() == dst.data_ptr() and p.stride() == dst.stride():
                continue
            p = as_act(p, dtype)
            sp, lds_ = _pl(p)
            dp, ldd = _pl(dst)
            lib.mte_copy_channels(sp, lds_, dp, ldd, B * H * W, c, _dt(p), st)
        if inv is not None:
            dst = buf[:, off:off + 8]
            dp, ldd = _pl(dst)
            lib.mte_upsample_inv_fwd(inv.contiguous().data_ptr(), dp, ldd, B, H // 2, W // 2, _dt(buf), st)
        ctx.chans = chans
        ctx.has_inv = inv is not None
        ctx.slots = [getattr(p, "_mte_fork_slot", None) for p in parts]
        return buf

    @staticmethod
    def backward(ctx, dbuf):
        dbuf = as_act(dbuf)
        B, _, H, W = dbuf.shape
        outs = []
        off = 0
        for c, slot in zip(ctx.chans, ctx.slots):
            g = dbuf[:, off:off + c]
            if slot is not None and slot["buf"] is None and _fork_target(slot["parent"], g.shape, g.dtype) is None:
                slot["buf"] = g
            outs.append(g)
            off += c
        dinv = None
        if ctx.has_inv:
            dinv = torch.empty((B, 1, H // 2, W // 2), dtype=torch.float32, device=dbuf.device)
            src = dbuf[:, off:off + 8]
            sp, lds_ = _pl(src)
            lib.mte_upsample_inv_bwd(sp, lds_, dinv.data_ptr(), B, H // 2, W // 2, 0, _dt(dbuf), _stream())
        return (dinv, None) + tuple(outs)


def new_concat_buffer(B, chans, with_inv, H, W, dtype=None, device="cuda"):
    c = sum(chans) + (8 if with_inv else 0)
    ld = (c + 31) // 32 * 32
    if ld == c or os.environ.get("MTE_CONCAT_TIGHT"):
        return new_act(B, c, H, W, dtype or compute_dtype(), device)
    return alias_of(new_act(B, ld, H, W, dtype or compute_dtype(), device)[:, :c])


def image_to_act(rgb, flip=False, dtype=None):
    _require_gpu(rgb)
    B, C, H, W = rgb.shape
    rgb = rgb.contiguous().float()
    out = new_act(B, round8(C), H, W, dtype or compute_dtype(), rgb.device)
    op, ldo = _pl(out)
    lib.mte_nchw_to_nhwc(rgb.data_ptr(), op, ldo, B, C, H, W, round8(C), 1 if flip else 0, _dt(out), _stream())
    return out




from .kernels_loss import EdgeLossFn, EdgeLossKindFn, BilinearResizeFn, DepthLossesFn, DepthLossesPairFn, SilogFn, SupervisedLossFn, NearestUpsampleFn, _EdgeScale, adam_step_flat, adamw_step_flat, sgd_step_flat
```

Measured before the change: 371.2 images/sec.

## Replace packing border band convolutions with ring-correction GEMMs on folded conv output

The packing layer previously recomputed its image borders by running separate unfolded 3D-pack and conv passes on band strips, then copying the strips into the output. It now runs only the folded conv over the whole image and applies an additive border correction. The correction is built from thin ring tensors (a 3-tap K3 projection of edge pixels) multiplied by negated edge-tap weights, plus a precomputed bias-correction table. Backward mirrors this with gather, ring GEMMs, class sums and scatter kernels, which removes the band dgrad/wgrad convolutions and rect copies. The cost is a new, complex kernel file whose index math must match the original padding semantics exactly.

```diff
diff --git a/include/mte_kernels.h b/include/mte_kernels.h
--- a/include/mte_kernels.h
+++ b/include/mte_kernels.h
@@ -101,6 +101,22 @@
 typedef struct { const void* src; long lds_; int Hs, Ws, sy, sx; void* dst; long ldd; int Hd, Wd, dy, dx, h, w, mode; } mte_rect_op;
 int mte_copy_rects(const void* ops, int n, int B, int C, int dtype, mte_stream_t stream);
 
+long mte_pack_ring_work_elems(void);
+long mte_pack_border_scatter_work_elems(int Co, int k);
+long mte_pack_border_class_sums_elems(int Co, int k);
+int mte_pack_ring_fwd(const void* P, long ldp, const float* K3, void* R_rows, void* R_cols, int B, int H2, int W2, int D, int dtype, mte_stream_t stream);
+int mte_pack_ring_bwd_data(const void* dR_rows, const void* dR_cols, const float* K3, void* dx, long lddx, int B, int H2, int W2, int D, int dtype,
+                           mte_stream_t stream);
+int mte_pack_ring_bwd_weight(const void* dR_rows, const void* dR_cols, const void* P, long ldp, float* dk3, float* work, int B, int H2, int W2, int D,
+                             int dtype, mte_stream_t stream);
+int mte_pack_border_weights(const float* W, const float* b3, float* Wr, float* Wc, float* Dt, int Co, int D, int k, mte_stream_t stream);
+int mte_pack_border_apply(void* y, long ldy, const float* corr_rows, const float* corr_cols, const float* Dt, int B, int H2, int W2, int Co, int k,
+                          int dtype, mte_stream_t stream);
+int mte_pack_border_gather(const void* dy, long lddy, void* G_rows, void* G_cols, int B, int H2, int W2, int Co, int k, int dtype, mte_stream_t stream);
+int mte_pack_border_class_sums(const void* dy, long lddy, float* part, int B, int H2, int W2, int Co, int k, int dtype, mte_stream_t stream);
+int mte_pack_border_scatter(const float* dWr, const float* dWc, const float* part, const float* W, const float* b3, float* dW, float* dk3b, float* work,
+                            int Co, int D, int k, mte_stream_t stream);
+
 int mte_invdepth_fwd(const void* x, long ldx, const float* w, const float* bias, float* out,
                      int B, int H, int W, int C, float min_depth, int dtype, mte_stream_t stream);
 int mte_invdepth_bwd_data(const float* w, const float* inv_out, const float* dout, float* dlogit,
diff --git a/mindtheedge_amd/_build.py b/mindtheedge_amd/_build.py
--- a/mindtheedge_amd/_build.py
+++ b/mindtheedge_amd/_build.py
@@ -6,7 +6,7 @@
 
 CSRC = os.path.join(os.path.dirname(os.path.abspath(__file__)), "csrc")
 LIB = os.path.join(CSRC, "libmte_hip.so")
-SOURCES = ["conv_igemm.hip", "conv_igemm8.hip", "conv_wgrad9.hip", "tap_wgrad.hip", "conv_patch.hip", "conv_stem.hip", "norm_act.hip", "pack3d.hip", "pack_fold.hip", "heads_misc.hip", "optim.hip", "edge_loss.hip", "edge_loss_kinds.hip", "supervised_loss.hip", "eval_metrics.hip", "dee_post.hip", "chamfer.hip", "canny.hip", "edge_match.hip", "san.hip", "data_prep.hip", "batch_prep.hip", "eval_prep.hip", "image_prep.hip", "lidar_prep.hip", "depth_viz.hip"]
+SOURCES = ["conv_igemm.hip", "conv_igemm8.hip", "conv_wgrad9.hip", "tap_wgrad.hip", "conv_patch.hip", "conv_stem.hip", "norm_act.hip", "pack3d.hip", "pack_fold.hip", "pack_border.hip", "heads_misc.hip", "optim.hip", "edge_loss.hip", "edge_loss_kinds.hip", "supervised_loss.hip", "eval_metrics.hip", "dee_post.hip", "chamfer.hip", "canny.hip", "edge_match.hip", "san.hip", "data_prep.hip", "batch_prep.hip", "eval_prep.hip", "image_prep.hip", "lidar_prep.hip", "depth_viz.hip"]
 FLAGS = ["--offload-arch=gfx950", "-O3", "-fPIC", "-std=c++17", "-Wno-unused-value", "-ffp-contract=off"]
 
 
diff --git a/mindtheedge_amd/_lib.py b/mindtheedge_amd/_lib.py
--- a/mindtheedge_amd/_lib.py
+++ b/mindtheedge_amd/_lib.py
@@ -20,7 +20,8 @@
 RETURNS = {}
 QUERIES = ("mte_conv2d_patch_supported", "mte_conv2d_stem_supported", "mte_conv2d_patch_wgrad_supported", "mte_conv2d_wgrad_nine_tap", "mte_conv2d_patch_fwd_gn_elems", "mte_conv2d_patch_pack_elems", "mte_depth_metrics_workspace_bytes",
            "mte_chamfer_workspace_bytes", "mte_edge_match_workspace_bytes", "mte_edge_loss_sums_elems", "mte_gn_fwd_is_single_pass", "mte_gn_fwd_is_single_pass_b",
-           "mte_edge_loss_work_elems", "mte_edge_loss_pair_work_elems", "mte_edge_loss_kind_work_elems", "mte_supervised_loss_work_elems", "mte_rank1_conv_bwd_records_elems", "mte_conv2d_patch_fwd_rank1_ok", "mte_gn_stats_elems", "mte_device_error_poll", "mte_invdepth_bwd_weight_workspace_elems", "mte_sparse_site_list_workspace_elems", "mte_image_resample_work_bytes", "mte_lidar_perturb_work_bytes", "mte_order_stats_work_bytes")
+           "mte_edge_loss_work_elems", "mte_edge_loss_pair_work_elems", "mte_edge_loss_kind_work_elems", "mte_supervised_loss_work_elems", "mte_rank1_conv_bwd_records_elems", "mte_conv2d_patch_fwd_rank1_ok", "mte_gn_stats_elems", "mte_device_error_poll", "mte_invdepth_bwd_weight_workspace_elems", "mte_sparse_site_list_workspace_elems", "mte_image_resample_work_bytes", "mte_lidar_perturb_work_bytes", "mte_order_stats_work_bytes",
+           "mte_pack_ring_work_elems", "mte_pack_border_scatter_work_elems", "mte_pack_border_class_sums_elems")
 
 
 def parse_header(path=HEADER, dev=False):
diff --git a/mindtheedge_amd/csrc/pack_border.hip b/mindtheedge_amd/csrc/pack_border.hip
--- /dev/null
+++ b/mindtheedge_amd/csrc/pack_border.hip
@@ -0,0 +1,472 @@
+#include "common.hpp"
+#include "pack_border_plan.hpp"
+
+namespace {
+
+inline int bgrid(long n, int cap = 4096) { long g = (n + 255) / 256; return (int)(g > cap ? cap : (g < 1 ? 1 : g)); }
+
+template <typename T>
+__device__ __forceinline__ void load_span(const T* __restrict__ p, int d0, int D, float* v) {
+    constexpr int P = Elem<T>::PER16;
+    v[0] = d0 > 0 ? Elem<T>::ld(p + d0 - 1) : 0.f;
+    v[33] = d0 + 32 < D ? Elem<T>::ld(p + d0 + 32) : 0.f;
+#pragma unroll
+    for (int c = 0; c < 32 / P; ++c) unpack16<T>(*(const u32x4_t*)(p + d0 + c * P), v + 1 + c * P);
+}
+template <typename T>
+__device__ __forceinline__ void store32(T* __restrict__ p, const float* v) {
+    constexpr int P = Elem<T>::PER16;
+#pragma unroll
+    for (int c = 0; c < 32 / P; ++c) *(u32x4_t*)(p + c * P) = pack16<T>(v + c * P);
+}
+
+__device__ __forceinline__ void ring_item(long it, int B, int H2, int W2, int nb, int* e, int* b, int* i, int* jb) {
+    const long per_row = (long)B * (W2 + 2) * nb, per_col = (long)B * H2 * nb;
+    int ee = 0;
+    if (it >= 2 * per_row) { it -= 2 * per_row; ee = 2; if (it >= per_col) { it -= per_col; ee = 3; } }
+    else if (it >= per_row) { it -= per_row; ee = 1; }
+    *e = ee;
+    *jb = (int)(it % nb); it /= nb;
+    const int len = pb_edge_len(ee, H2, W2);
+    *i = (int)(it % len); *b = (int)(it / len);
+}
+
+template <typename T>
+__global__ __launch_bounds__(256) void ring_fwd_kernel(const T* __restrict__ P, long ldp, const float* __restrict__ K3, T* __restrict__ Rr, T* __restrict__ Rc,
+                                                       int B, int H2, int W2, int D) {
+    __shared__ float s3[108];
+    if (threadIdx.x < 108) s3[threadIdx.x] = K3[threadIdx.x];
+    __syncthreads();
+    const int nb = D / 32;
+    const long total = 2L * B * (W2 + 2 + H2) * nb;
+    for (long it = blockIdx.x * (long)blockDim.x + threadIdx.x; it < total; it += (long)gridDim.x * blockDim.x) {
+        int e, b, i, jb;
+        ring_item(it, B, H2, W2, nb, &e, &b, &i, &jb);
+        const int d0 = 32 * jb, len = pb_edge_len(e, H2, W2);
+        float in[3][34];
+#pragma unroll
+        for (int a = 0; a < 3; ++a) {
+            int h, w;
+            if (pb_edge_src(e, i, a, H2, W2, &h, &w)) load_span<T>(P + (((long)b * H2 + h) * W2 + w) * ldp, d0, D, in[a]);
+            else {
+#pragma unroll
+                for (int q = 0; q < 34; ++q) in[a][q] = 0.f;
+            }
+        }
+        T* out = (e < 2 ? Rr : Rc) + (((long)(e & 1) * B + b) * len + i) * 4 * D + d0;
+        for (int f = 0; f < 4; ++f) {
+            float acc[32];
+#pragma unroll
+            for (int q = 0; q < 32; ++q) acc[q] = 0.f;
+#pragma unroll
+            for (int a = 0; a < 3; ++a)
+#pragma unroll
+                for (int kd = 0; kd < 3; ++kd) {
+                    const float kv = s3[pb_k3_index(e, f, kd, a)];
+#pragma unroll
+                    for (int q = 0; q < 32; ++q) acc[q] = fmaf(kv, in[a][q + kd], acc[q]);
+                }
+            store32<T>(out + (long)f * D, acc);
+        }
+    }
+}
+
+template <typename T>
+__global__ __launch_bounds__(256) void ring_bwd_data_kernel(const T* __restrict__ dRr, const T* __restrict__ dRc, const float* __restrict__ K3,
+                                                            T* __restrict__ dx, long lddx, int B, int H2, int W2, int D) {
+    constexpr int P = Elem<T>::PER16;
+    __shared__ float s3[108];
+    if (threadIdx.x < 108) s3[threadIdx.x] = K3[threadIdx.x];
+    __syncthreads();
+    const int nb = D / 32;
+    const long npix = pb_border_count(H2, W2, 1);
+    const long total = (long)B * npix * nb * 4;
+    for (long i4 = blockIdx.x * (long)blockDim.x + threadIdx.x; i4 < total; i4 += (long)gridDim.x * blockDim.x) {
+        const int f = (int)(i4 & 3); const long it = i4 >> 2;
+        const int jb = (int)(it % nb); long t = it / nb;
+        const long pix = t % npix; const int b = (int)(t / npix);
+        int h, w;
+        pb_border_pixel(pix, H2, W2, 1, &h, &w);
+        const int d0 = 32 * jb;
+        float acc[32];
+#pragma unroll
+        for (int q = 0; q < 32; ++q) acc[q] = 0.f;
+        for (int e = 0; e < 4; ++e) {
+            int along, off;
+            if (!pb_edge_of_pixel(e, h, w, H2, W2, &along, &off)) continue;
+            const int len = pb_edge_len(e, H2, W2);
+            const T* base = (e < 2 ? dRr : dRc) + ((long)(e & 1) * B + b) * len * 4 * D + (long)f * D;
+            for (int a = 0; a < 3; ++a) {
+                const int i = along + off - a;
+                if (i < 0 || i >= len) continue;
+                float v[34];
+                load_span<T>(base + (long)i * 4 * D, d0, D, v);
+#pragma unroll
+                for (int kd = 0; kd < 3; ++kd) {
+                    const float kv = s3[pb_k3_index(e, f, kd, a)];
+#pragma unroll
+                    for (int q = 0; q < 32; ++q) acc[q] = fmaf(kv, v[q - kd + 2], acc[q]);
+                }
+            }
+        }
+#pragma unroll
+        for (int q = 0; q < 32; ++q) {
+            acc[q] += __shfl_xor(acc[q], 1, 64);
+            acc[q] += __shfl_xor(acc[q], 2, 64);
+        }
+        const int s = f;
+        T* p = dx + (((long)b * 2 * H2 + 2 * h + (s >> 1)) * 2 * W2 + 2 * w + (s & 1)) * lddx + 8 * jb;
+        float cur[8];
+        unpack16<T>(*(const u32x4_t*)p, cur);
+        if constexpr (P == 4) unpack16<T>(*(const u32x4_t*)(p + 4), cur + 4);
+#pragma unroll
+        for (int c = 0; c < 8; ++c) {
+            float a_ = 0.f;
+#pragma unroll
+            for (int ss = 0; ss < 4; ++ss) a_ = ss == s ? acc[4 * c + ss] : a_;
+            cur[c] += a_;
+        }
+        *(u32x4_t*)p = pack16<T>(cur);
+        if constexpr (P == 4) *(u32x4_t*)(p + 4) = pack16<T>(cur + 4);
+    }
+}
+
+template <typename T>
+__global__ __launch_bounds__(256) void ring_bwd_weight_kernel(const T* __restrict__ dRr, const T* __restrict__ dRc, const T* __restrict__ P, long ldp,
+                                                              float* __restrict__ part, int B, int H2, int W2, int D) {
+    constexpr int PE = Elem<T>::PER16;
+    __shared__ float sred[4][36];
+    const int e = blockIdx.y, nb = D / 32, len = pb_edge_len(e, H2, W2);
+    const T* dR = e < 2 ? dRr : dRc;
+    float acc[36];
+#pragma unroll
+    for (int q = 0; q < 36; ++q) acc[q] = 0.f;
+    const long total = (long)B * len * nb;
+    for (long it = blockIdx.x * (long)blockDim.x + threadIdx.x; it < total; it += (long)gridDim.x * blockDim.x) {
+        const int jb = (int)(it % nb); long t = it / nb;
+        const int i = (int)(t % len), b = (int)(t / len), d0 = 32 * jb;
+        float in[3][34];
+#pragma unroll
+        for (int a = 0; a < 3; ++a) {
+            int h, w;
+            if (pb_edge_src(e, i, a, H2, W2, &h, &w)) load_span<T>(P + (((long)b * H2 + h) * W2 + w) * ldp, d0, D, in[a]);
+            else {
+#pragma unroll
+                for (int q = 0; q < 34; ++q) in[a][q] = 0.f;
+            }
+        }
+        const T* g = dR + (((long)(e & 1) * B + b) * len + i) * 4 * D + d0;
+#pragma unroll
+        for (int f = 0; f < 4; ++f) {
+            float gv[32];
+#pragma unroll
+            for (int c = 0; c < 32 / PE; ++c) unpack16<T>(*(const u32x4_t*)(g + (long)f * D + c * PE), gv + c * PE);
+#pragma unroll
+            for (int kd = 0; kd < 3; ++kd)
+#pragma unroll
+                for (int a = 0; a < 3; ++a) {
+                    float s = acc[(f * 3 + kd) * 3 + a];
+#pragma unroll
+                    for (int q = 0; q < 32; ++q) s = fmaf(gv[q], in[a][q + kd], s);
+                    acc[(f * 3 + kd) * 3 + a] = s;
+                }
+        }
+    }
+    const int lane = threadIdx.x & 63, wave = threadIdx.x >> 6;
+#pragma unroll
+    for (int q = 0; q < 36; ++q) {
+        const float s = wave_sum(acc[q]);
+        if (lane == 0) sred[wave][q] = s;
+    }
+    __syncthreads();
+    if (threadIdx.x < 36)
+        part[((long)e * gridDim.x + blockIdx.x) * 36 + threadIdx.x] = (sred[0][threadIdx.x] + sred[1][threadIdx.x]) + (sred[2][threadIdx.x] + sred[3][threadIdx.x]);
+}
+
+static_assert(PB_RING_BLOCKS == 64, "ring_bwd_weight_finish_kernel: one lane per workgroup of partials");
+__global__ __launch_bounds__(64) void ring_bwd_weight_finish_kernel(const float* __restrict__ part, float* __restrict__ dk3) {
+    const int t = blockIdx.x, lane = threadIdx.x;
+    const int dw = t % 3, dh = (t / 3) % 3, fk = t / 9;
+    float sum = 0.f;
+    for (int e = 0; e < 4; ++e) {
+        const int fix = (e == 0 || e == 2) ? 2 : 0;
+        int a;
+        if (e < 2) { if (dh != fix) continue; a = dw; }
+        else { if (dw != fix) continue; a = dh; }
+        sum += part[((long)e * PB_RING_BLOCKS + lane) * 36 + fk * 3 + a];
+    }
+    sum = wave_sum(sum);
+    if (lane == 0) dk3[t] += sum;
+}
+
+__global__ __launch_bounds__(256) void border_weights_kernel(const float* __restrict__ W, const float* __restrict__ b3, float* __restrict__ Wr,
+                                                             float* __restrict__ Wc, float* __restrict__ Dt, int Co, int D, int k) {
+    const int pad = k >> 1, CT = 4 * D, kk = k * k;
+    const long half = 2L * pad * Co * CT * k;
+    for (long idx = blockIdx.x * (long)blockDim.x + threadIdx.x; idx < 2 * half; idx += (long)gridDim.x * blockDim.x) {
+        const bool cols = idx >= half;
+        long r = cols ? idx - half : idx;
+        const int t = (int)(r % k); r /= k;
+        const int ch = (int)(r % CT); r /= CT;
+        const int co = (int)(r % Co); const int fj = (int)(r / Co);
+        const int tap = pb_tap(fj / pad, fj % pad, pad);
+        const float* wp = W + ((long)co * CT + ch) * kk;
+        if (cols) Wc[idx - half] = -wp[t * k + tap];
+        else Wr[idx] = -wp[tap * k + t];
+    }
+    __shared__ float sS[32], sw[4];
+    const int lane = threadIdx.x & 63, wave = threadIdx.x >> 6, nc = 2 * pad + 1;
+    for (int co = blockIdx.x; co < Co; co += gridDim.x) {
+        for (int t = 0; t < kk; ++t) {
+            float a = 0.f;
+            for (int ch = threadIdx.x; ch < CT; ch += 256) a = fmaf(b3[ch / D], W[((long)co * CT + ch) * kk + t], a);
+            a = wave_sum(a);
+            __syncthreads();
+            if (lane == 0) sw[wave] = a;
+            __syncthreads();
+            if (threadIdx.x == 0) sS[t] = (sw[0] + sw[1]) + (sw[2] + sw[3]);
+        }
+        __syncthreads();
+        if ((int)threadIdx.x < nc * nc) {
+            const int cy = threadIdx.x / nc, cx = threadIdx.x % nc;
+            float s = 0.f;
+            for (int t = 0; t < kk; ++t)
+                if (pb_tap_outside(cy, t / k, pad) || pb_tap_outside(cx, t % k, pad)) s += sS[t];
+            Dt[(long)threadIdx.x * Co + co] = -s;
+        }
+        __syncthreads();
+    }
+}
+
+template <typename T>
+__global__ __launch_bounds__(256) void border_apply_kernel(T* __restrict__ y, long ldy, const float* __restrict__ cr, const float* __restrict__ cc,
+                                                           const float* __restrict__ Dt, int B, int H2, int W2, int Co, int pad) {
+    constexpr int P = Elem<T>::PER16;
+    const int cpr = Co / P, N = 2 * pad * Co, nc = 2 * pad + 1;
+    const long npix = pb_border_count(H2, W2, pad), total = (long)B * npix * cpr;
+    for (long it = blockIdx.x * (long)blockDim.x + threadIdx.x; it < total; it += (long)gridDim.x * blockDim.x) {
+        const int c0 = (int)(it % cpr) * P; long t = it / cpr;
+        const long pix = t % npix; const int b = (int)(t / npix);
+        int r, x;
+        pb_border_pixel(pix, H2, W2, pad, &r, &x);
+        T* p = y + (((long)b * H2 + r) * W2 + x) * ldy + c0;
+        float v[P], add[P];
+        unpack16<T>(*(const u32x4_t*)p, v);
+#pragma unroll
+        for (int c = 0; c < P; ++c) add[c] = 0.f;
+        const float* src[4] = {nullptr, nullptr, nullptr, nullptr};
+        if (r < pad) src[0] = cr + (((long)b * (W2 + 2)) + x + 1) * N + pb_col(0, r, c0, pad, Co);
+        if (H2 - 1 - r < pad) src[1] = cr + (((long)(B + b) * (W2 + 2)) + x + 1) * N + pb_col(1, H2 - 1 - r, c0, pad, Co);
+        if (x < pad) src[2] = cc + (((long)b * H2) + r) * N + pb_col(0, x, c0, pad, Co);
+        if (W2 - 1 - x < pad) src[3] = cc + (((long)(B + b) * H2) + r) * N + pb_col(1, W2 - 1 - x, c0, pad, Co);
+#pragma unroll
+        for (int s = 0; s < 4; ++s)
+            if (src[s]) {
+#pragma unroll
+                for (int c = 0; c < P; c += 4) {
+                    const f32x4_t q = *(const f32x4_t*)(src[s] + c);
+                    add[c] += q[0]; add[c + 1] += q[1]; add[c + 2] += q[2]; add[c + 3] += q[3];
+                }
+            }
+        const float* dt = Dt + (long)(pb_class(r, H2, pad) * nc + pb_class(x, W2, pad)) * Co + c0;
+#pragma unroll
+        for (int c = 0; c < P; ++c) v[c] += add[c] + dt[c];
+        *(u32x4_t*)p = pack16<T>(v);
+    }
+}
+
+template <typename T>
+__global__ __launch_bounds__(256) void border_gather_kernel(const T* __restrict__ dy, long lddy, T* __restrict__ Gr, T* __restrict__ Gc,
+                                                            int B, int H2, int W2, int Co, int pad) {
+    constexpr int P = Elem<T>::PER16;
+    const int N = 2 * pad * Co, npr = N / P;
+    const long rows = 2L * B * (W2 + 2) * npr, total = rows + 2L * B * H2 * npr;
+    for (long it = blockIdx.x * (long)blockDim.x + threadIdx.x; it < total; it += (long)gridDim.x * blockDim.x) {
+        const bool cols = it >= rows;
+        long t = cols ? it - rows : it;
+        const int n0 = (int)(t % npr) * P; t /= npr;
+        const int len = cols ? H2 : W2 + 2;
+        const int i = (int)(t % len), fb = (int)(t / len), far = fb / B, b = fb % B;
+        const int fj = n0 / Co, co = n0 % Co, j = fj % pad;
+        u32x4_t v = {0u, 0u, 0u, 0u};
+        if (fj / pad == far) {
+            if (cols) v = *(const u32x4_t*)(dy + (((long)b * H2 + i) * W2 + (far ? W2 - 1 - j : j)) * lddy + co);
+            else if (i >= 1 && i <= W2) v = *(const u32x4_t*)(dy + (((long)b * H2 + (far ? H2 - 1 - j : j)) * W2 + i - 1) * lddy + co);
+        }
+        *(u32x4_t*)((cols ? Gc : Gr) + ((long)fb * len + i) * N + n0) = v;
+    }
+}
+
+template <typename T>
+__global__ __launch_bounds__(256) void border_class_sums_kernel(const T* __restrict__ dy, long lddy, float* __restrict__ part,
+                                                                int B, int H2, int W2, int Co, int pad) {
+    __shared__ float sred[4][64];
+    const int nc = 2 * pad + 1, cls = blockIdx.y, cy = cls / nc, cx = cls % nc, split = blockIdx.x;
+    const int lane = threadIdx.x & 63, wave = threadIdx.x >> 6;
+    const bool centre = cy == pad && cx == pad;
+    const int ny = pb_class_count(cy, H2, pad), nx = pb_class_count(cx, W2, pad), y0 = pb_class_first(cy, H2, pad), x0 = pb_class_first(cx, W2, pad);
+    const long np = centre ? 0 : (long)B * ny * nx;
+    for (int c0 = 0; c0 < Co; c0 += 64) {
+        const int c = c0 + lane;
+        float a = 0.f;
+        if (c < Co)
+#pragma unroll 4
+            for (long p = split * 4 + wave; p < np; p += 4 * PB_CLASS_SPLITS) {
+                const int x = (int)(p % nx); long t = p / nx;
+                const int yy = (int)(t % ny), b = (int)(t / ny);
+                a += Elem<T>::ld(dy + (((long)b * H2 + y0 + yy) * W2 + x0 + x) * lddy + c);
+            }
+        __syncthreads();
+        sred[wave][lane] = a;
+        __syncthreads();
+        if (wave == 0 && c < Co) part[((long)cls * PB_CLASS_SPLITS + split) * Co + c] = (sred[0][lane] + sred[1][lane]) + (sred[2][lane] + sred[3][lane]);
+    }
+}
+
+__global__ __launch_bounds__(256) void border_ds_kernel(const float* __restrict__ part, float* __restrict__ dS, int Co, int k) {
+    const int pad = k >> 1, nc = 2 * pad + 1, kk = k * k;
+    const int lane = threadIdx.x & 63, idx = blockIdx.x * 4 + (threadIdx.x >> 6);
+    if (idx >= Co * kk) return;
+    const int t = idx % kk, co = idx / kk;
+    float s = 0.f;
+    for (int q = lane; q < nc * nc * PB_CLASS_SPLITS; q += 64) {
+        const int cls = q / PB_CLASS_SPLITS;
+        if (pb_tap_outside(cls / nc, t / k, pad) || pb_tap_outside(cls % nc, t % k, pad)) s += part[(long)q * Co + co];
+    }
+    s = wave_sum(s);
+    if (lane == 0) dS[idx] = -s;
+}
+
+__global__ __launch_bounds__(256) void border_scatter_kernel(const float* __restrict__ dWr, const float* __restrict__ dWc, const float* __restrict__ dS,
+                                                             const float* __restrict__ W, const float* __restrict__ b3, float* __restrict__ dW,
+                                                             float* __restrict__ part3, int Co, int D, int k) {
+    __shared__ float sred[4][4];
+    const int pad = k >> 1, CT = 4 * D, kk = k * k;
+    const long total = (long)Co * CT * kk;
+    float a0 = 0.f, a1 = 0.f, a2 = 0.f, a3 = 0.f;
+    for (long idx = blockIdx.x * (long)blockDim.x + threadIdx.x; idx < total; idx += (long)gridDim.x * blockDim.x) {
+        const int t = (int)(idx % kk); long r = idx / kk;
+        const int ch = (int)(r % CT), co = (int)(r / CT), ty = t / k, tx = t - ty * k, f = ch / D;
+        const float ds = dS[co * kk + t];
+        float v = 0.f;
+        int far, j;
+        if (pb_tap_owner(ty, pad, &far, &j)) v -= dWr[((long)pb_col(far, j, co, pad, Co) * CT + ch) * k + tx];
+        if (pb_tap_owner(tx, pad, &far, &j)) v -= dWc[((long)pb_col(far, j, co, pad, Co) * CT + ch) * k + ty];
+        dW[idx] = fmaf(b3[f], ds, v);
+        const float c = ds * W[idx];
+        a0 += f == 0 ? c : 0.f; a1 += f == 1 ? c : 0.f; a2 += f == 2 ? c : 0.f; a3 += f == 3 ? c : 0.f;
+    }
+    const int lane = threadIdx.x & 63, wave = threadIdx.x >> 6;
+    a0 = wave_sum(a0); a1 = wave_sum(a1); a2 = wave_sum(a2); a3 = wave_sum(a3);
+    if (lane == 0) { sred[wave][0] = a0; sred[wave][1] = a1; sred[wave][2] = a2; sred[wave][3] = a3; }
+    __syncthreads();
+    if (threadIdx.x < 4) part3[(long)blockIdx.x * 4 + threadIdx.x] = (sred[0][threadIdx.x] + sred[1][threadIdx.x]) + (sred[2][threadIdx.x] + sred[3][threadIdx.x]);
+}
+
+constexpr int SCATTER_BLOCKS = 256;
+
+__global__ __launch_bounds__(64) void border_scatter_finish_kernel(const float* __restrict__ part3, float* __restrict__ db3) {
+    const int f = blockIdx.x, lane = threadIdx.x;
+    float s = 0.f;
+    for (int blk = lane; blk < SCATTER_BLOCKS; blk += 64) s += part3[(long)blk * 4 + f];
+    s = wave_sum(s);
+    if (lane == 0) db3[f] += s;
+}
+
+inline bool ring_ok(int B, int H2, int W2, int D, int dtype) {
+    return B > 0 && H2 >= 2 && W2 >= 2 && D > 0 && D % 32 == 0 && (dtype == MTE_DT_BF16 || dtype == MTE_DT_F32);
+}
+inline bool border_ok(int B, int H2, int W2, int Co, int k, int dtype) {
+    return B > 0 && Co > 0 && Co % 8 == 0 && k <= 5 && pb_shape_ok(H2, W2, k) && (dtype == MTE_DT_BF16 || dtype == MTE_DT_F32);
+}
+
+}
+
+extern "C" {
+
+long mte_pack_ring_work_elems(void) { return 4L * PB_RING_BLOCKS * 36; }
+long mte_pack_border_scatter_work_elems(int Co, int k) { return (long)Co * k * k + 4L * SCATTER_BLOCKS; }
+long mte_pack_border_class_sums_elems(int Co, int k) { return (long)k * k * PB_CLASS_SPLITS * Co; }
+
+int mte_pack_ring_fwd(const void* P, long ldp, const float* K3, void* R_rows, void* R_cols, int B, int H2, int W2, int D, int dtype, hipStream_t stream) {
+    (void)hipGetLastError();
+    if (!P || !K3 || !R_rows || !R_cols || !ring_ok(B, H2, W2, D, dtype) || ldp < D || ldp % (dtype == MTE_DT_BF16 ? 8 : 4) != 0) return MTE_ERR_ARG;
+    const int grid = bgrid(2L * B * (W2 + 2 + H2) * (D / 32));
+    if (dtype == MTE_DT_BF16) hipLaunchKernelGGL(ring_fwd_kernel<bf16_t>, dim3(grid), dim3(256), 0, stream, (const bf16_t*)P, ldp, K3, (bf16_t*)R_rows, (bf16_t*)R_cols, B, H2, W2, D);
+    else hipLaunchKernelGGL(ring_fwd_kernel<float>, dim3(grid), dim3(256), 0, stream, (const float*)P, ldp, K3, (float*)R_rows, (float*)R_cols, B, H2, W2, D);
+    return mte_check_launch();
+}
+
+int mte_pack_ring_bwd_data(const void* dR_rows, const void* dR_cols, const float* K3, void* dx, long lddx, int B, int H2, int W2, int D, int dtype,
+                           hipStream_t stream) {
+    (void)hipGetLastError();
+    if (!dR_rows || !dR_cols || !K3 || !dx || !ring_ok(B, H2, W2, D, dtype) || lddx < D / 4 || lddx % (dtype == MTE_DT_BF16 ? 8 : 4) != 0) return MTE_ERR_ARG;
+    const int grid = bgrid((long)B * pb_border_count(H2, W2, 1) * (D / 32) * 4);
+    if (dtype == MTE_DT_BF16) hipLaunchKernelGGL(ring_bwd_data_kernel<bf16_t>, dim3(grid), dim3(256), 0, stream, (const bf16_t*)dR_rows, (const bf16_t*)dR_cols, K3, (bf16_t*)dx, lddx, B, H2, W2, D);
+    else hipLaunchKernelGGL(ring_bwd_data_kernel<float>, dim3(grid), dim3(256), 0, stream, (const float*)dR_rows, (const float*)dR_cols, K3, (float*)dx, lddx, B, H2, W2, D);
+    return mte_check_launch();
+}
+
+int mte_pack_ring_bwd_weight(const void* dR_rows, const void* dR_cols, const void* P, long ldp, float* dk3, float* work, int B, int H2, int W2, int D,
+                             int dtype, hipStream_t stream) {
+    (void)hipGetLastError();
+    if (!dR_rows || !dR_cols || !P || !dk3 || !work || !ring_ok(B, H2, W2, D, dtype) || ldp < D || ldp % (dtype == MTE_DT_BF16 ? 8 : 4) != 0) return MTE_ERR_ARG;
+    const dim3 grid(PB_RING_BLOCKS, 4);
+    if (dtype == MTE_DT_BF16) hipLaunchKernelGGL(ring_bwd_weight_kernel<bf16_t>, grid, dim3(256), 0, stream, (const bf16_t*)dR_rows, (const bf16_t*)dR_cols, (const bf16_t*)P, ldp, work, B, H2, W2, D);
+    else hipLaunchKernelGGL(ring_bwd_weight_kernel<float>, grid, dim3(256), 0, stream, (const float*)dR_rows, (const float*)dR_cols, (const float*)P, ldp, work, B, H2, W2, D);
+    hipLaunchKernelGGL(ring_bwd_weight_finish_kernel, dim3(108), dim3(64), 0, stream, (const float*)work, dk3);
+    return mte_check_launch();
+}
+
+int mte_pack_border_weights(const float* W, const float* b3, float* Wr, float* Wc, float* Dt, int Co, int D, int k, hipStream_t stream) {
+    (void)hipGetLastError();
+    if (!W || !b3 || !Wr || !Wc || !Dt || Co <= 0 || D <= 0 || (k & 1) == 0 || k < 3 || k > 5) return MTE_ERR_ARG;
+    int grid = bgrid(4L * (k / 2) * Co * 4 * D * k);
+    if (grid < Co) grid = Co < 4096 ? Co : 4096;
+    hipLaunchKernelGGL(border_weights_kernel, dim3(grid), dim3(256), 0, stream, W, b3, Wr, Wc, Dt, Co, D, k);
+    return mte_check_launch();
+}
+
+int mte_pack_border_apply(void* y, long ldy, const float* corr_rows, const float* corr_cols, const float* Dt, int B, int H2, int W2, int Co, int k,
+                          int dtype, hipStream_t stream) {
+    (void)hipGetLastError();
+    if (!y || !corr_rows || !corr_cols || !Dt || !border_ok(B, H2, W2, Co, k, dtype) || ldy < Co || ldy % (dtype == MTE_DT_BF16 ? 8 : 4) != 0) return MTE_ERR_ARG;
+    const int pad = k / 2, per16 = dtype == MTE_DT_BF16 ? 8 : 4;
+    const int grid = bgrid((long)B * pb_border_count(H2, W2, pad) * (Co / per16));
+    if (dtype == MTE_DT_BF16) hipLaunchKernelGGL(border_apply_kernel<bf16_t>, dim3(grid), dim3(256), 0, stream, (bf16_t*)y, ldy, corr_rows, corr_cols, Dt, B, H2, W2, Co, pad);
+    else hipLaunchKernelGGL(border_apply_kernel<float>, dim3(grid), dim3(256), 0, stream, (float*)y, ldy, corr_rows, corr_cols, Dt, B, H2, W2, Co, pad);
+    return mte_check_launch();
+}
+
+int mte_pack_border_gather(const void* dy, long lddy, void* G_rows, void* G_cols, int B, int H2, int W2, int Co, int k, int dtype, hipStream_t stream) {
+    (void)hipGetLastError();
+    if (!dy || !G_rows || !G_cols || !border_ok(B, H2, W2, Co, k, dtype) || lddy < Co || lddy % (dtype == MTE_DT_BF16 ? 8 : 4) != 0) return MTE_ERR_ARG;
+    const int pad = k / 2, per16 = dtype == MTE_DT_BF16 ? 8 : 4;
+    const int grid = bgrid(2L * B * (W2 + 2 + H2) * (2 * pad * Co / per16));
+    if (dtype == MTE_DT_BF16) hipLaunchKernelGGL(border_gather_kernel<bf16_t>, dim3(grid), dim3(256), 0, stream, (const bf16_t*)dy, lddy, (bf16_t*)G_rows, (bf16_t*)G_cols, B, H2, W2, Co, pad);
+    else hipLaunchKernelGGL(border_gather_kernel<float>, dim3(grid), dim3(256), 0, stream, (const float*)dy, lddy, (float*)G_rows, (float*)G_cols, B, H2, W2, Co, pad);
+    return mte_check_launch();
+}
+
+int mte_pack_border_class_sums(const void* dy, long lddy, float* part, int B, int H2, int W2, int Co, int k, int dtype, hipStream_t stream) {
+    (void)hipGetLastError();
+    if (!dy || !part || !border_ok(B, H2, W2, Co, k, dtype) || lddy < Co) return MTE_ERR_ARG;
+    const dim3 grid(PB_CLASS_SPLITS, k * k);
+    if (dtype == MTE_DT_BF16) hipLaunchKernelGGL(border_class_sums_kernel<bf16_t>, grid, dim3(256), 0, stream, (const bf16_t*)dy, lddy, part, B, H2, W2, Co, k / 2);
+    else hipLaunchKernelGGL(border_class_sums_kernel<float>, grid, dim3(256), 0, stream, (const float*)dy, lddy, part, B, H2, W2, Co, k / 2);
+    return mte_check_launch();
+}
+
+int mte_pack_border_scatter(const float* dWr, const float* dWc, const float* part, const float* W, const float* b3, float* dW, float* dk3b, float* work,
+                            int Co, int D, int k, hipStream_t stream) {
+    (void)hipGetLastError();
+    if (!dWr || !dWc || !part || !W || !b3 || !dW || !dk3b || !work || Co <= 0 || D <= 0 || (k & 1) == 0 || k < 3 || k > 5) return MTE_ERR_ARG;
+    float* dS = work;
+    float* part3 = work + (long)Co * k * k;
+    hipLaunchKernelGGL(border_ds_kernel, dim3((Co * k * k + 3) / 4), dim3(256), 0, stream, part, dS, Co, k);
+    hipLaunchKernelGGL(border_scatter_kernel, dim3(SCATTER_BLOCKS), dim3(256), 0, stream, dWr, dWc, (const float*)dS, W, b3, dW, part3, Co, D, k);
+    hipLaunchKernelGGL(border_scatter_finish_kernel, dim3(4), dim3(64), 0, stream, (const float*)part3, dk3b + 108);
+    return mte_check_launch();
+}
+
+}
diff --git a/mindtheedge_amd/csrc/pack_border_plan.hpp b/mindtheedge_amd/csrc/pack_border_plan.hpp
--- /dev/null
+++ b/mindtheedge_amd/csrc/pack_border_plan.hpp
@@ -0,0 +1,48 @@
+#pragma once
+
+#ifndef PB_HD
+#ifdef __HIPCC__
+#define PB_HD __host__ __device__ inline
+#else
+#define PB_HD inline
+#endif
+#endif
+
+#define PB_CLASS_SPLITS 64
+#define PB_RING_BLOCKS 64
+
+PB_HD int pb_edge_len(int e, int H2, int W2) { return e < 2 ? W2 + 2 : H2; }
+PB_HD bool pb_edge_src(int e, int i, int a, int H2, int W2, int* h, int* w) {
+    if (e < 2) { *h = e == 0 ? 0 : H2 - 1; *w = i + a - 2; return *w >= 0 && *w < W2; }
+    *w = e == 2 ? 0 : W2 - 1; *h = i + a - 1; return *h >= 0 && *h < H2;
+}
+PB_HD int pb_k3_index(int e, int f, int kd, int a) {
+    const int fix = (e == 0 || e == 2) ? 2 : 0;
+    return e < 2 ? ((f * 3 + kd) * 3 + fix) * 3 + a : ((f * 3 + kd) * 3 + a) * 3 + fix;
+}
+PB_HD bool pb_edge_of_pixel(int e, int h, int w, int H2, int W2, int* along, int* off) {
+    if (e < 2) { *along = w; *off = 2; return h == (e == 0 ? 0 : H2 - 1); }
+    *along = h; *off = 1; return w == (e == 2 ? 0 : W2 - 1);
+}
+
+PB_HD int pb_tap(int far, int j, int pad) { return far ? pad + 1 + j : pad - 1 - j; }
+PB_HD int pb_col(int far, int j, int co, int pad, int Co) { return (far * pad + j) * Co + co; }
+PB_HD bool pb_tap_owner(int t, int pad, int* far, int* j) {
+    if (t == pad) return false;
+    *far = t > pad; *j = t > pad ? t - pad - 1 : pad - 1 - t;
+    return true;
+}
+PB_HD int pb_class(int r, int n, int pad) { return r < pad ? r : (n - 1 - r < pad ? 2 * pad - (n - 1 - r) : pad); }
+PB_HD bool pb_tap_outside(int cls, int t, int pad) { return cls < pad ? t < pad - cls : (cls > pad ? t > 3 * pad - cls : false); }
+PB_HD int pb_class_count(int cls, int n, int pad) { return cls == pad ? n - 2 * pad : 1; }
+PB_HD int pb_class_first(int cls, int n, int pad) { return cls < pad ? cls : (cls == pad ? pad : n - 1 - (2 * pad - cls)); }
+
+PB_HD long pb_border_count(int H2, int W2, int pad) { return 2L * pad * W2 + 2L * pad * (H2 - 2 * pad); }
+PB_HD void pb_border_pixel(long idx, int H2, int W2, int pad, int* r, int* x) {
+    const long rows = 2L * pad * W2;
+    if (idx < rows) { const int q = (int)(idx / W2); *x = (int)(idx % W2); *r = q < pad ? q : H2 - 2 * pad + q; return; }
+    idx -= rows;
+    const int q = (int)(idx % (2 * pad));
+    *r = pad + (int)(idx / (2 * pad)); *x = q < pad ? q : W2 - 2 * pad + q;
+}
+PB_HD bool pb_shape_ok(int H2, int W2, int k) { return (k & 1) && k >= 3 && H2 >= 2 * (k / 2) && W2 >= 2 * (k / 2); }
diff --git a/mindtheedge_amd/kernels.py b/mindtheedge_amd/kernels.py
--- a/mindtheedge_amd/kernels.py
+++ b/mindtheedge_amd/kernels.py
@@ -589,21 +589,6 @@
     lib.set_option(3, 1 if flag else 0, lazy=True)
 
 
-class _BandChain:
-
-    def __enter__(self):
-        return self
-
-    def __exit__(self, *exc):
-        return False
-
-    def mark(self):
-        return None
-
-    def join(self, ev=None):
-        return None
-
-
 def join_side_stream():
     if _side["dirty"]:
         for st in _side["streams"]:
@@ -1128,39 +1113,6 @@
         return dx, dw3, db3, None
 
 
-def _rect(src, sy, sx, dst, dy, dx, h, w, mode=0):
-    B, C, Hd, Wd = dst.shape
-    dp, ldd = _pl(dst)
-    if mode == 2:
-        lib.mte_copy_rect(0, 0, 0, 0, 0, 0, dp, ldd, Hd, Wd, dy, dx, B, h, w, C, 2, _dt(dst), _stream())
-        return
-    sp, lds_ = _pl(src)
-    lib.mte_copy_rect(sp, lds_, src.shape[2], src.shape[3], sy, sx, dp, ldd, Hd, Wd, dy, dx, B, h, w, C, mode, _dt(dst), _stream())
-
-
-class _RectOp(ctypes.Structure):
-    _fields_ = [("src", ctypes.c_void_p), ("lds_", ctypes.c_long), ("Hs", ctypes.c_int), ("Ws", ctypes.c_int), ("sy", ctypes.c_int),
-                ("sx", ctypes.c_int), ("dst", ctypes.c_void_p), ("ldd", ctypes.c_long), ("Hd", ctypes.c_int), ("Wd", ctypes.c_int),
-                ("dy", ctypes.c_int), ("dx", ctypes.c_int), ("h", ctypes.c_int), ("w", ctypes.c_int), ("mode", ctypes.c_int)]
-
-
-def _rects(ops):
-    arr = (_RectOp * len(ops))()
-    B = C = dt = None
-    for o, (src, sy, sx, dst, dy, dx, h, w, mode) in zip(arr, ops):
-        Bd, Cd, Hd, Wd = dst.shape
-        if B is None:
-            B, C, dt = Bd, Cd, _dt(dst)
-        elif (Bd, Cd, _dt(dst)) != (B, C, dt):
-            raise MteError("rectangle batch: mixed batch / channel / dtype")
-        dp, ldd = _pl(dst)
-        o.dst, o.ldd, o.Hd, o.Wd, o.dy, o.dx, o.h, o.w, o.mode = dp, ldd, Hd, Wd, dy, dx, h, w, mode
-        if mode != 2:
-            sp, lds_ = _pl(src)
-            o.src, o.lds_, o.Hs, o.Ws, o.sy, o.sx = sp, lds_, src.shape[2], src.shape[3], sy, sx
-    lib.mte_copy_rects(ctypes.addressof(arr), len(ops), B, C, dt, _stream())
-
-
 def _deliver(p, t):
     sk = _sink["active"]
     if sk is not None:
@@ -1235,6 +1187,8 @@
 
 def pack_fold_applicable(H2, W2, k):
     hb = 2 * (k // 2) + 1
+    if k > 5:
+        return False
     return H2 > 2 * hb and W2 > 2 * hb and (2.0 * hb / H2 + 2.0 * hb / W2) <= _cfg["pack_fold_max_overhead"]
 
 
@@ -1244,8 +1198,10 @@
 
 def _fold_now(f, w, w3, b, b3):
     co, C4, k = f["geom"]
-    lib.mte_fold_pack_weights(w.detach().data_ptr(), w3.detach().contiguous().float().data_ptr(), b.detach().data_ptr(),
-                              b3.detach().contiguous().float().data_ptr(), f["Wf"].data_ptr(), f["bf"].data_ptr(), co, C4, k, _stream())
+    w3c, b3c = w3.detach().contiguous().float(), b3.detach().contiguous().float()
+    lib.mte_fold_pack_weights(w.detach().data_ptr(), w3c.data_ptr(), b.detach().data_ptr(), b3c.data_ptr(), f["Wf"].data_ptr(), f["bf"].data_ptr(),
+                              co, C4, k, _stream())
+    lib.mte_pack_border_weights(w.detach().data_ptr(), b3c.data_ptr(), f["Wr"].data_ptr(), f["Wc"].data_ptr(), f["Dt"].data_ptr(), co, C4, k, _stream())
     f["key"] = _fold_key(w, w3, b, b3)
 
 
@@ -1254,12 +1210,16 @@
     if f is None or f["geom"] != (co, 4 * C, k) or f["Wf"].device != dev:
         f = pack_fold.fold = {"geom": (co, 4 * C, k), "key": None,
                               "Wf": torch.empty((co, 4 * C, k + 2, k + 2), dtype=torch.float32, device=dev),
-                              "bf": torch.empty((co,), dtype=torch.float32, device=dev)}
+                              "bf": torch.empty((co,), dtype=torch.float32, device=dev),
+                              "Wr": torch.empty((2 * (k // 2) * co, 16 * C, 1, k), dtype=torch.float32, device=dev),
+                              "Wc": torch.empty((2 * (k // 2) * co, 16 * C, k, 1), dtype=torch.float32, device=dev),
+                              "Dt": torch.empty((k * k, co), dtype=torch.float32, device=dev),
+                              "pk_r": WeightPack(), "pk_c": WeightPack()}
         _fold_hooks.append(weakref.ref(pack_fold))
     f["params"] = tuple(weakref.ref(t) for t in (w, w3, b, b3))
     if f["key"] != _fold_key(w, w3, b, b3) or _FOLD_INLINE:
         _fold_now(f, w, w3, b, b3)
-        pack_fold.key = None
+        pack_fold.key = f["pk_r"].key = f["pk_c"].key = None
     return f["Wf"], f["bf"]
 
 
@@ -1308,6 +1268,35 @@
     return True
 
 
+def _ring_gemm(x, wpack, cout, kh, kw, out_f32, flags=0):
+    Bl, Cp, H, W = x.shape
+    xp, ldx = _pl(x)
+    if out_f32:
+        out = torch.empty((Bl, H * W, cout), dtype=torch.float32, device=x.device)
+        op, ldo = out.data_ptr(), cout
+    else:
+        out = new_act(Bl, cout, H, W, x.dtype, x.device)
+        op, ldo = _pl(out)
+    ws, ws_n = _splitk_workspace(Bl * H * W, cout, x.device)
+    lib.mte_conv2d_igemm(xp, ldx, wpack.data_ptr(), 0, op, ldo, 1 if out_f32 else 0, Bl, H, W, Cp, cout, kh, kw, _dt(x), _ptr(ws), ws_n, flags, _stream())
+    return out
+
+
+def _ring_wgrad(x, g, w):
+    cout, cin, kh, kw = w.shape
+    Bl, Cp, H, W = x.shape
+    xp, ldx = _pl(x)
+    gp, ldg = _pl(g)
+    per = cout * kh * kw * Cp
+    cap = max(1, min(32, (96 << 20) // (4 * per)))
+    stage = torch.empty((cap, cout, kh * kw, Cp), dtype=torch.float32, device=x.device)
+    parts = ctypes.c_int(1)
+    lib.mte_conv2d_wgrad(xp, ldx, gp, ldg, stage.data_ptr(), cap, ctypes.byref(parts), Bl, H, W, Cp, cout, kh, kw, _dt(x), _stream())
+    dw = torch.empty((cout, cin, kh, kw), dtype=torch.float32, device=x.device)
+    lib.mte_unpack_conv_wgrad(stage.data_ptr(), parts.value, dw.data_ptr(), cout, cin, kh, kw, Cp, _stream())
+    return dw
+
+
 class PackFoldedConvGnEluFn(torch.autograd.Function):
 
     @staticmethod
@@ -1315,37 +1304,28 @@
         B, C, H, W = x.shape
         H2, W2 = H // 2, W // 2
         co, _, k, _ = w.shape
-        pad, hb = k // 2, 2 * (k // 2) + 1
+        pad, N = k // 2, 2 * (k // 2) * co
         dt, dev = _dt(x), x.device
         w3c, b3c = w3.detach().contiguous().float(), b3.detach().contiguous().float()
-        bands = _BandChain()
-        with bands:
-            wu, _ = pack_unf.get(w, x.dtype, False)
-            xb1 = new_act(2 * B, C, 2 * hb, W, x.dtype, dev)
-            xb2 = new_act(2 * B, C, H, 2 * hb, x.dtype, dev)
-            _rects([(x, 0, 0, xb1[:B], 0, 0, 2 * hb, W, 0), (x, H - 2 * hb, 0, xb1[B:], 0, 0, 2 * hb, W, 0),
-                    (x, 0, 0, xb2[:B], 0, 0, H, 2 * hb, 0), (x, 0, W - 2 * hb, xb2[B:], 0, 0, H, 2 * hb, 0)])
-            Tb = []
-            for xb, (hh, ww) in ((xb1, (hb, W2)), (xb2, (H2, hb))):
-                T = new_act(2 * B, 16 * C, hh, ww, x.dtype, dev)
-                sp, lds_ = _pl(xb)
-                tp, ldt = _pl(T)
-                lib.mte_pack3d_fwd(sp, lds_, w3c.data_ptr(), b3c.data_ptr(), tp, ldt, 2 * B, xb.shape[2], xb.shape[3], C, dt, _stream())
-                Tb.append(T)
-            yb1 = conv_forward(Tb[0], wu, b, co, k, k, pack=pack_unf, w=w)
-            yb2 = conv_forward(Tb[1], wu, b, co, k, k, pack=pack_unf, w=w)
         P = new_act(B, 4 * C, H2, W2, x.dtype, dev)
         xp, ldx = _pl(x)
         pp, ldp = _pl(P)
         lib.mte_pixel_shuffle(xp, ldx, pp, ldp, B, H, W, C, 0, dt, _stream())
         Wf, bf = _folded_weights(pack_fold, w, w3, b, b3, co, C, k, dev)
+        f = pack_fold.fold
         wfp, _ = pack_fold.get(Wf, x.dtype, False)
         y = conv_forward(P, wfp, bf, co, k + 2, k + 2, pack=pack_fold, w=Wf)
-        bands.join()
-        _rects([(yb1[:B], 0, 0, y, 0, 0, pad, W2, 0), (yb1[B:], hb - pad, 0, y, H2 - pad, 0, pad, W2, 0),
-                (yb2[:B], pad, 0, y, pad, 0, H2 - 2 * pad, pad, 0), (yb2[B:], pad, hb - pad, y, pad, W2 - pad, H2 - 2 * pad, pad, 0)])
+        Rr = new_act(2 * B, 16 * C, 1, W2 + 2, x.dtype, dev)
+        Rc = new_act(2 * B, 16 * C, H2, 1, x.dtype, dev)
+        lib.mte_pack_ring_fwd(pp, ldp, w3c.data_ptr(), Rr.data_ptr(), Rc.data_ptr(), B, H2, W2, 4 * C, dt, _stream())
+        wr, _ = f["pk_r"].get(f["Wr"], x.dtype, False)
+        wc, _ = f["pk_c"].get(f["Wc"], x.dtype, False)
+        cr = _ring_gemm(Rr, wr, N, 1, k, True, _CONV_SOLO)
+        cc = _ring_gemm(Rc, wc, N, k, 1, True, _CONV_SOLO)
+        yp, ldy = _pl(y)
+        lib.mte_pack_border_apply(yp, ldy, cr.data_ptr(), cc.data_ptr(), f["Dt"].data_ptr(), B, H2, W2, co, k, dt, _stream())
         z, stats = _gn_forward(y, None, None, gamma, beta, GN_EPS, out=None if out is None else alias_of(out))
-        ctx.save_for_backward(P, xb1, xb2, Tb[0], Tb[1], y, stats, w, w3c, b3c, gamma, beta, Wf)
+        ctx.save_for_backward(P, Rr, Rc, y, stats, w, w3c, b3c, gamma, beta, Wf)
         ctx.params = (w3, b3, b)
         ctx.packs = (pack_unf, pack_fold)
         ctx.geom = (B, C, H, W, co, k)
@@ -1353,79 +1333,63 @@
 
     @staticmethod
     def backward(ctx, dz):
-        P, xb1, xb2, T1, T2, y, stats, w, w3c, b3c, gamma, beta, Wf = ctx.saved_tensors
+        P, Rr, Rc, y, stats, w, w3c, b3c, gamma, beta, Wf = ctx.saved_tensors
         w3, b3, b = ctx.params
         pack_unf, pack_fold = ctx.packs
         B, C, H, W, co, k = ctx.geom
-        H2, W2, pad, hb = H // 2, W // 2, k // 2, 2 * (k // 2) + 1
+        H2, W2, pad, N = H // 2, W // 2, k // 2, 2 * (k // 2) * co
         dt, dev = _dt(P), P.device
+        f = pack_fold.fold
         gg, sg = _grad_dst(gamma, zero=True)
         gbt, sbt = _grad_dst(beta, zero=True)
         dy, _, dgamma, dbeta = _gn_backward(dz, y, None, None, stats, gamma, beta, GN_EPS, False, dgamma=gg, dbeta=gbt)
-        bands = _BandChain()
-        with bands:
-            dyb1 = torch.zeros((2 * B, hb, W2, co), dtype=P.dtype, device=dev).permute(0, 3, 1, 2)
-            dyb2 = torch.zeros((2 * B, H2, hb, co), dtype=P.dtype, device=dev).permute(0, 3, 1, 2)
-            _rects([(dy, 0, 0, dyb1[:B], 0, 0, pad, W2, 0), (dy, H2 - pad, 0, dyb1[B:], hb - pad, 0, pad, W2, 0),
-                    (dy, pad, 0, dyb2[:B], pad, 0, H2 - 2 * pad, pad, 0), (dy, pad, W2 - pad, dyb2[B:], pad, hb - pad, H2 - 2 * pad, pad, 0)])
-            gathered = bands.mark()
-            dTs, dxb = [], []
-            for xb, T, dyb in ((xb1, T1, dyb1), (xb2, T2, dyb2)):
-                dT, _, _ = conv_backward(T, dyb, w, pack_unf, True, need_dw=False)
-                Bb, _, hx, wx = xb.shape
-                tp, ldt = _pl(dT)
-                dxi = new_act(Bb, C, hx, wx, P.dtype, dev)
-                dp_, ldd = _pl(dxi)
-                lib.mte_pack3d_bwd_data(tp, ldt, w3c.data_ptr(), dp_, ldd, Bb, hx, wx, C, dt, _stream())
-                dTs.append(dT)
-                dxb.append(dxi)
-        bands.join(gathered)
-        _rects([(None, 0, 0, dy, 0, 0, pad, W2, 2), (None, 0, 0, dy, H2 - pad, 0, pad, W2, 2),
-                (None, 0, 0, dy, pad, 0, H2 - 2 * pad, pad, 2), (None, 0, 0, dy, pad, W2 - pad, H2 - 2 * pad, pad, 2)])
+        dyp, lddy = _pl(dy)
+        pp, ldp = _pl(P)
+        Gr = new_act(2 * B, N, 1, W2 + 2, P.dtype, dev)
+        Gc = new_act(2 * B, N, H2, 1, P.dtype, dev)
+        lib.mte_pack_border_gather(dyp, lddy, Gr.data_ptr(), Gc.data_ptr(), B, H2, W2, co, k, dt, _stream())
+        _, wrb = f["pk_r"].get(f["Wr"], P.dtype, True)
+        _, wcb = f["pk_c"].get(f["Wc"], P.dtype, True)
+        dRr = _ring_gemm(Gr, wrb, 16 * C, 1, k, False)
+        dRc = _ring_gemm(Gc, wcb, 16 * C, k, 1, False)
 
         def weight_grads():
-            bands.join()
             sw = _stream()
-            dw_band = db_band = None
             dst3 = _claim_adjacent(w3, b3)
             dk3b = dst3 if dst3 is not None else torch.zeros((112,), dtype=torch.float32, device=dev)
             gw_dst, gw_sunk = _grad_dst(w)
             gb_dst, gb_sunk = _grad_dst(b)
-            for xb, T, dyb, dT in ((xb1, T1, dyb1, dTs[0]), (xb2, T2, dyb2, dTs[1])):
-                dwi, dbi = _conv_wgrad(T, dyb, w, True, gw_dst if dw_band is None else None, None)
-                dw_band = dwi if dw_band is None else dw_band.add_(dwi)
-                db_band = dbi if db_band is None else db_band.add_(dbi)
-                Bb, _, hx, wx = xb.shape
-                tmp = torch.empty((112,), dtype=torch.float32, device=dev)
-                sp, lds_ = _pl(xb)
-                tp, ldt = _pl(dT)
-                lib.mte_pack3d_bwd_weight(sp, lds_, tp, ldt, tmp.data_ptr(), Bb, hx, wx, C, dt, sw)
-                dk3b.add_(tmp)
-            dWf, dbf = _conv_wgrad(P, dy, Wf, True, None, None)
-            lib.mte_unfold_pack_wgrad(dWf.data_ptr(), dbf.data_ptr(), w.detach().data_ptr(), w3c.data_ptr(), b3c.data_ptr(),
-                                      dw_band.data_ptr(), dk3b.data_ptr(), co, 4 * C, k, 1, sw)
-            db = torch.add(dbf, db_band, out=gb_dst)
+            part = torch.empty((int(lib.mte_pack_border_class_sums_elems(co, k)),), dtype=torch.float32, device=dev)
+            lib.mte_pack_border_class_sums(dyp, lddy, part.data_ptr(), B, H2, W2, co, k, dt, sw)
+            dWr = _ring_wgrad(Rr, Gr, f["Wr"])
+            dWc = _ring_wgrad(Rc, Gc, f["Wc"])
+            work = torch.empty((int(lib.mte_pack_border_scatter_work_elems(co, k)) + int(lib.mte_pack_ring_work_elems()),), dtype=torch.float32, device=dev)
+            lib.mte_pack_border_scatter(dWr.data_ptr(), dWc.data_ptr(), part.data_ptr(), w.detach().data_ptr(), b3c.data_ptr(), gw_dst.data_ptr(),
+                                        dk3b.data_ptr(), work.data_ptr(), co, 4 * C, k, sw)
+            lib.mte_pack_ring_bwd_weight(dRr.data_ptr(), dRc.data_ptr(), pp, ldp, dk3b.data_ptr(),
+                                         work.data_ptr() + 4 * int(lib.mte_pack_border_scatter_work_elems(co, k)), B, H2, W2, 4 * C, dt, sw)
+            dWf, db = _conv_wgrad(P, dy, Wf, True, None, gb_dst)
+            lib.mte_unfold_pack_wgrad(dWf.data_ptr(), db.data_ptr(), w.detach().data_ptr(), w3c.data_ptr(), b3c.data_ptr(),
+                                      gw_dst.data_ptr(), dk3b.data_ptr(), co, 4 * C, k, 1, sw)
             if dst3 is not None:
                 _announce(w3, b3)
                 g3 = gb3 = None
             else:
                 g3, gb3 = _deliver_pair(w3, b3, dk3b, 108)
-            return (g3, gb3, _grad_ret(w, dw_band, gw_sunk), _grad_ret(b, db, gb_sunk))
+            return (g3, gb3, _grad_ret(w, gw_dst, gw_sunk), _grad_ret(b, db, gb_sunk))
 
         if _side["enabled"] and _all_sunk(w3, b3, w, b):
-            with torch.cuda.stream(_side_stream_for(P, dy, T1, T2, dyb1, dyb2, dTs[0], dTs[1], xb1, xb2, Wf)):
+            with torch.cuda.stream(_side_stream_for(P, dy, Rr, Rc, Gr, Gc, dRr, dRc, Wf)):
                 g3, gb3, gw, gb = weight_grads()
         else:
             g3, gb3, gw, gb = weight_grads()
         dx = new_act(B, C, H, W, P.dtype, dev)
+        dxp, lddx = _pl(dx)
         if not _dgrad_unshuffled(dy, Wf, pack_fold, dx, k + 2):
             dP, _, _ = conv_backward(P, dy, Wf, pack_fold, True, need_dw=False)
             sp, lds_ = _pl(dP)
-            dp_, ldd = _pl(dx)
-            lib.mte_pixel_shuffle(sp, lds_, dp_, ldd, B, H, W, C, 1, dt, _stream())
-        bands.join()
-        _rects([(dxb[0][:B], 0, 0, dx, 0, 0, 2 * hb, W, 1), (dxb[0][B:], 0, 0, dx, H - 2 * hb, 0, 2 * hb, W, 1)])
-        _rects([(dxb[1][:B], 0, 0, dx, 0, 0, H, 2 * hb, 1), (dxb[1][B:], 0, 0, dx, 0, W - 2 * hb, H, 2 * hb, 1)])
+            lib.mte_pixel_shuffle(sp, lds_, dxp, lddx, B, H, W, C, 1, dt, _stream())
+        lib.mte_pack_ring_bwd_data(dRr.data_ptr(), dRc.data_ptr(), w3c.data_ptr(), dxp, lddx, B, H2, W2, 4 * C, dt, _stream())
         return (dx, g3, gb3, gw, gb, _grad_ret(gamma, dgamma, sg), _grad_ret(beta, dbeta, sbt), None, None, None)
 
 
```

Result: faster. 378.1 images/sec (median of 6 runs) (+1.9%).
